# zhm1205/Multimodal_TTA

Hardware: AMD Instinct MI355X
Metric: adapted volumes/sec (higher is better)
Workload: dtype bf16

## Files before the change

### include/mmtta.h

```cpp
#ifndef MMTTA_H
#define MMTTA_H

#include <stdint.h>

#ifdef __cplusplus
extern "C" {
#endif

#define MMTTA_ABI_VERSION 2

typedef enum {
  MMTTA_OK = 0,
  MMTTA_ERR_INVALID = -1,
  MMTTA_ERR_UNSUPPORTED = -2,
  MMTTA_ERR_LAUNCH = -3,
  MMTTA_ERR_WORKSPACE = -4
} mmtta_status;

typedef enum { MMTTA_F32 = 0, MMTTA_BF16 = 1 } mmtta_dtype;

typedef struct {
  void* ptr;
  int32_t n, c, d, h, w;
  int64_t sn, sc, sd, sh, sw;
  int32_t dtype;
  int32_t flags;
} mmtta_tensor;

#define MMTTA_TENSOR_OWNS_PAD 1

#define MMTTA_ACT_NONE 0
#define MMTTA_ACT_RELU 1
#define MMTTA_ACT_LEAKY_RELU 2
typedef struct {
  const float* mean;
  const float* rstd;
  const float* gamma;
  const float* beta;
  int32_t relu;
  int32_t per_item;
  const float* scale;
  const float* shift;
  float negative_slope;
  int32_t _pad2;
} mmtta_norm_on_load;

const char* mmtta_last_error(void);
int mmtta_abi_version(void);

#define MMTTA_OPT_PROFILE_MAIN_KERNEL_ONLY 1
#define MMTTA_OPT_SPLITK_BELOW 2
#define MMTTA_OPT_SPLITK_TARGET 3
#define MMTTA_OPT_WGRAD_WORKGROUPS 4
#define MMTTA_OPT_WGRAD_THIN_SLABS 5
#define MMTTA_OPT_IGEMM_PIPELINE 6
#define MMTTA_OPT_EPILOGUE_VEC16 9
#define MMTTA_OPT_IGEMM_LEAN 10
#define MMTTA_OPT_WGRAD_VECTOR_STAGING 11
#define MMTTA_OPT_CLASS_FUSED_MIN_WORKGROUPS 12
#define MMTTA_OPT_THIN_MFMA 13
#define MMTTA_OPT_IGEMM_FRAGMENT_REUSE 14
#define MMTTA_OPT_LAME_TILED 15
#define MMTTA_OPT_RAW_STAGING 16
#define MMTTA_OPT_HEAD_LOSS_PAIR 17
#define MMTTA_OPT_THIN_LEAN 18
#define MMTTA_OPT_WGRAD_EPILOGUE_UPDATE 19
#define MMTTA_OPT_CLS8_PIPELINE 20
#define MMTTA_OPT_CLS8_LEAN_EPILOGUE 21
int mmtta_set_option(int key, int value);

int mmtta_copy_strided(const mmtta_tensor* src, const mmtta_tensor* dst, void* stream);

typedef enum {
  MMTTA_CONV_FWD = 0,
  MMTTA_CONV_DGRAD = 1,
  MMTTA_CONVT_FWD = 2,
  MMTTA_CONVT_DGRAD = 3
} mmtta_conv_op;

typedef struct {
  int32_t op;
  int32_t ksize;
  int32_t stride;
  int32_t cin;
  int32_t cout;
  int32_t dtype;
} mmtta_conv_desc;

int64_t mmtta_conv_packed_bytes(const mmtta_conv_desc* desc);

int mmtta_conv_pack_weights(const mmtta_conv_desc* desc, const float* w_master, void* packed, void* stream);

typedef struct {
  mmtta_conv_desc desc;
  const float* w_master;
  void* packed;
} mmtta_pack_item;
int64_t mmtta_conv_pack_table_bytes(int count);
int mmtta_conv_pack_table_build(const mmtta_pack_item* items, int count, void* table_host, int64_t* total);
int mmtta_conv_pack_batched(const void* table_dev, int count, int64_t total, void* stream);

typedef struct {
  int32_t tiles;
  int32_t launches;
  int32_t ksplit;
  int32_t stats_rows;
  int32_t config;
  int32_t _pad;
  int64_t workspace_bytes;
} mmtta_conv_plan_t;

int mmtta_conv_plan(const mmtta_conv_desc* desc, const mmtta_tensor* x, const mmtta_tensor* y,
                    mmtta_conv_plan_t* plan);

typedef struct {
  const mmtta_tensor* add;
  mmtta_norm_on_load add_norm;
} mmtta_conv_epilogue;

int mmtta_conv_run(const mmtta_conv_desc* desc, const mmtta_tensor* x, const mmtta_norm_on_load* x_norm,
                   const void* packed, const float* bias, const mmtta_conv_epilogue* epi,
                   const mmtta_tensor* y, int accumulate, float* stats, void* workspace,
                   int64_t workspace_bytes, void* stream);

int mmtta_conv_route(const mmtta_conv_desc* desc, const mmtta_tensor* x, const mmtta_norm_on_load* x_norm,
                     const mmtta_conv_epilogue* epi, const mmtta_tensor* y, int accumulate, const float* stats);

int mmtta_conv_stages_raw(const mmtta_conv_desc* desc, const mmtta_tensor* x, const mmtta_norm_on_load* x_norm,
                          const mmtta_conv_epilogue* epi, const mmtta_tensor* y, int accumulate, const float* stats);

int mmtta_conv_cls8_pipelined(const mmtta_conv_desc* desc, const mmtta_tensor* x, const mmtta_norm_on_load* x_norm,
                              const mmtta_conv_epilogue* epi, const mmtta_tensor* y, int accumulate, const float* stats);

int mmtta_conv_cls8_lean_epilogue(const mmtta_conv_desc* desc, const mmtta_tensor* x, const mmtta_norm_on_load* x_norm,
                                  const mmtta_conv_epilogue* epi, const mmtta_tensor* y, int accumulate, const float* stats);

int mmtta_conv_thin_lean(const mmtta_conv_desc* desc, const mmtta_tensor* x, const mmtta_norm_on_load* x_norm,
                         const mmtta_conv_epilogue* epi, const mmtta_tensor* y, int accumulate, const float* stats);

int mmtta_conv_thin_kernel(const mmtta_conv_desc* desc, const mmtta_tensor* x, const mmtta_norm_on_load* x_norm,
                           const mmtta_conv_epilogue* epi, const mmtta_tensor* y, int accumulate, const float* stats);

typedef struct {
  int32_t items_per_set;
  int32_t inner;
  int64_t packed_outer, packed_inner;
  int64_t weight_outer, weight_inner;
  int64_t bias_outer, bias_inner;
} mmtta_param_sets;

int mmtta_conv_run_sets(const mmtta_conv_desc* desc, const mmtta_tensor* x, const mmtta_norm_on_load* x_norm,
                        const void* packed, const float* bias, const mmtta_conv_epilogue* epi,
                        const mmtta_tensor* y, int accumulate, float* stats, void* workspace,
                        int64_t workspace_bytes, const mmtta_param_sets* sets, void* stream);

int mmtta_conv_head_loss_eligible(const mmtta_conv_desc* desc, const mmtta_tensor* x, const mmtta_norm_on_load* x_norm,
                                  const mmtta_conv_epilogue* epi, const mmtta_tensor* y, const mmtta_tensor* dlogits,
                                  int softmax, int per_item);
int64_t mmtta_conv_head_loss_partials(const mmtta_conv_desc* desc, const mmtta_tensor* x, const mmtta_tensor* y);
int mmtta_conv_head_loss_run_sets(const mmtta_conv_desc* desc, const mmtta_tensor* x, const mmtta_norm_on_load* x_norm,
                                  const void* packed, const float* bias, const mmtta_conv_epilogue* epi,
                                  const mmtta_tensor* y, const mmtta_tensor* dlogits, int softmax, int per_item,
                                  double* partial, float* loss, const mmtta_param_sets* sets, void* stream);

int64_t mmtta_conv_wgrad_workspace_bytes(const mmtta_conv_desc* desc, const mmtta_tensor* x,
                                         const mmtta_tensor* dy);
int mmtta_conv_wgrad_kernel(const mmtta_conv_desc* desc, const mmtta_tensor* x, const mmtta_tensor* dy);
int mmtta_conv_wgrad_stages_raw(const mmtta_conv_desc* desc, const mmtta_tensor* x, const mmtta_norm_on_load* x_norm,
                                const mmtta_tensor* dy);
int mmtta_conv_wgrad(const mmtta_conv_desc* desc, const mmtta_tensor* x, const mmtta_norm_on_load* x_norm,
                     const mmtta_tensor* dy, float* dw, float* db, int accumulate, void* workspace,
                     int64_t workspace_bytes, void* stream);

int64_t mmtta_conv_wgrad_workspace_bytes_sets(const mmtta_conv_desc* desc, const mmtta_tensor* x, const mmtta_tensor* dy,
                                              const mmtta_param_sets* sets);
int mmtta_conv_wgrad_sets(const mmtta_conv_desc* desc, const mmtta_tensor* x, const mmtta_norm_on_load* x_norm,
                          const mmtta_tensor* dy, float* dw, float* db, int accumulate, void* workspace,
                          int64_t workspace_bytes, const mmtta_param_sets* sets, void* stream);
int mmtta_conv_wgrad_plan_sets(const mmtta_conv_desc* desc, const mmtta_tensor* x, const mmtta_tensor* dy,
                               const mmtta_param_sets* sets, int32_t plan[4]);

typedef struct {
  int32_t clip, zscore, masked, min_count;
  float lo, hi, mask_gt, eps;
  float mean, std;
  int32_t legacy, _pad;
} mmtta_intensity_rule;
int64_t mmtta_intensity_scratch_bytes(int channels);
int mmtta_intensity_normalize(const mmtta_tensor* x, const mmtta_intensity_rule* rules, const mmtta_tensor* y,
                              void* scratch, void* stream);

typedef enum {
  MMTTA_NORM_INSTANCE = 0,
  MMTTA_NORM_BATCH = 1,
  MMTTA_NORM_GROUP = 2
} mmtta_norm_kind;

int mmtta_norm_stats_finalize(int kind, int groups, const float* part, int rows_per_n, int n, int c,
                              int64_t count, float eps, int training, float* running_mean,
                              float* running_var, float momentum, float* mean, float* rstd,
                              const float* gamma, const float* beta, float* scale, float* shift,
                              double* scratch, void* stream);

typedef struct {
  int32_t items_per_set;
  int32_t _pad;
  int64_t affine_stride;
  int64_t stats_stride;
} mmtta_norm_sets;

int mmtta_norm_stats_finalize_sets(int kind, int groups, const float* part, int rows_per_n, int n, int c,
                                   int64_t count, float eps, int training, float* running_mean,
                                   float* running_var, float momentum, float* mean, float* rstd,
                                   const float* gamma, const float* beta, float* scale, float* shift,
                                   float* gamma_items, float* beta_items, double* scratch,
                                   const mmtta_norm_sets* sets, void* stream);

int mmtta_reduce_rows_per_n(const mmtta_tensor* t);

int mmtta_channel_stats(const mmtta_tensor* x, float* part, void* stream);

// ... 76 lines not shown
int mmtta_entropy_loss_items(const mmtta_tensor* logits, int softmax, const mmtta_tensor* dlogits,
                             double* partial, float* loss, void* stream);

int64_t mmtta_entropy_filtered_partials(const mmtta_tensor* logits);
int mmtta_entropy_filtered_items(const mmtta_tensor* logits, int softmax, float margin, const uint8_t* keep_in,
                                 uint8_t* keep_out, const mmtta_tensor* dlogits, double* partial, float* loss,
                                 int64_t* kept, void* stream);

int mmtta_mirror_views(const mmtta_tensor* x, const mmtta_tensor* y, int views, const int32_t* view_axes, void* stream);
int64_t mmtta_memo_partials(const mmtta_tensor* logits, int views);
int mmtta_memo_loss_items(const mmtta_tensor* logits, int softmax, int views, const int32_t* view_axes,
                          const mmtta_tensor* dlogits, double* partial, float* loss, void* stream);
int mmtta_memo_ensemble(const mmtta_tensor* logits, int softmax, int views, const int32_t* view_axes,
                        const mmtta_tensor* out, void* stream);

int64_t mmtta_consistency_partials(const mmtta_tensor* logits);
int mmtta_consistency_loss_items(const mmtta_tensor* logits, const mmtta_tensor* target, int softmax,
                                 const mmtta_tensor* dlogits, double* partial, float* loss, void* stream);
int64_t mmtta_cotta_update_partials(int64_t n, int sets);
int mmtta_cotta_update_sets(float* w, float* teacher, const float* source, int64_t n, int sets, int64_t w_stride,
                            int64_t teacher_stride, double alpha, float restore_p, uint64_t seed, const int32_t* step,
                            const int32_t* ordinals, int64_t* partial, int64_t* restored, void* stream);

int mmtta_affine_views(const mmtta_tensor* x, const mmtta_tensor* y, int views, int first, int count,
                       const float* matrices_host, const float* matrices, void* stream);
int mmtta_affine_ensemble(const mmtta_tensor* logits, int softmax, int views, const int32_t* view_axes, int first, int count,
                          const float* inv_host, const float* inv, const mmtta_tensor* out, void* stream);

int mmtta_magnitude_select_class(int64_t length);
int64_t mmtta_magnitude_select_chunks(int64_t length);
int64_t mmtta_magnitude_select_scratch_bytes(int count, int sets);
int mmtta_magnitude_select_sets(const float* g, const int64_t* table, const int64_t* table_host, int count, int sets,
                                int64_t set_stride, uint32_t* gamma_out, void* scratch, void* stream);
int64_t mmtta_petal_update_partials(int64_t n, int sets);
int mmtta_petal_update_sets(float* w, float* teacher, const float* source, const float* g, const uint32_t* gamma,
                            const int64_t* table, const int64_t* table_host, int count, int64_t n, int sets,
                            int64_t w_stride, int64_t teacher_stride, int64_t g_stride, double alpha, int64_t* partial,
                            int64_t* restored, void* stream);

int64_t mmtta_intensity_range_partials(const mmtta_tensor* x);
int mmtta_intensity_range(const mmtta_tensor* x, float* partial, float* range, void* stream);
int mmtta_augment_views(const mmtta_tensor* x, const mmtta_tensor* y, int views, const int32_t* view_axes,
                        const float* table_host, const float* table, const float* range, uint64_t seed,
                        const int32_t* ordinals, void* stream);

int64_t mmtta_entropy_weighted_partials(const mmtta_tensor* logits);
int mmtta_entropy_weighted_items(const mmtta_tensor* logits, int softmax, float margin, uint8_t* keep_out,
                                 const mmtta_tensor* dlogits, double* partial, float* loss, int64_t* kept, void* stream);
int64_t mmtta_pseudo_label_partials(const mmtta_tensor* logits);
int mmtta_pseudo_label_loss_items(const mmtta_tensor* logits, int softmax, const mmtta_tensor* dlogits, double* partial,
                                  float* loss, void* stream);
int mmtta_fisher_accumulate_sets(float* fisher, const float* grads, int64_t n, int sets, int64_t set_stride, void* stream);
int mmtta_fisher_scale(float* fisher, int64_t n, float count, void* stream);
int64_t mmtta_fisher_penalty_partials(int64_t n, int sets);
int mmtta_fisher_penalty_sets(const float* w, float* g, const float* fisher, const float* source, int64_t n, int sets,
                              int replicas, int64_t set_stride, float lambda, double* partial, float* penalty, void* stream);

int mmtta_patch_shuffle(const mmtta_tensor* x, const mmtta_tensor* y, const int32_t* grid, const int32_t* table, void* stream);
int64_t mmtta_deyo_partials(const mmtta_tensor* logits);
int mmtta_deyo_loss_items(const mmtta_tensor* logits, const mmtta_tensor* logits_shuffled, const int32_t* grid,
                          const int32_t* table, int softmax, float margin, float margin0, float plpd_threshold,
                          uint8_t* keep_out, const mmtta_tensor* dlogits, double* partial, float* loss, int64_t* kept,
                          int64_t* kept_entropy, void* stream);

int mmtta_lame_refine(const mmtta_tensor* logits0, const mmtta_tensor* x, uint32_t channel_mask, int softmax, int connectivity,
                      float weight, float sigma, int iterations, const mmtta_tensor* work, const mmtta_tensor* out,
                      int64_t* flipped, void* stream);

int64_t mmtta_crf_partials(const mmtta_tensor* logits);
int mmtta_crf_entropy_items(const mmtta_tensor* logits, const mmtta_tensor* x, uint32_t channel_mask, int softmax,
                            int connectivity, int form, float weight, float sigma, const mmtta_tensor* dlogits,
                            double* partial, float* loss, float* entropy, float* pairwise, void* stream);

int64_t mmtta_nuclear_scratch(const mmtta_tensor* logits, int softmax, int bd, int bh, int bw);
int mmtta_nuclear_entropy_items(const mmtta_tensor* logits, int softmax, int bd, int bh, int bw, float entropy_weight,
                                float weight, float eps, const mmtta_tensor* dlogits, double* scratch, float* loss,
                                float* entropy, float* nuclear, void* stream);

typedef struct mmtta_input_norm_branch {
  const mmtta_tensor* dy;
  const float* weight;
  int64_t set_stride;
  int32_t ksize, stride;
} mmtta_input_norm_branch;
int mmtta_input_norm_apply(const mmtta_tensor* x, const mmtta_tensor* y, const float* theta, const float* range,
                           uint32_t keep_mask, int gamma, void* stream);
int64_t mmtta_input_norm_grad_partials(const mmtta_tensor* x);
int mmtta_input_norm_grad(const mmtta_tensor* x, const mmtta_input_norm_branch* branches, int n_branches, float* theta,
                          const float* range, uint32_t keep_mask, int gamma, double* partial, float* grad, float* exp_avg,
                          float* exp_avg_sq, int32_t* step, double lr, double bound_log_scale, double bound_shift,
                          double bound_log_gamma, void* stream);

#define MMTTA_BIAS_ANCHOR_MIN 0
#define MMTTA_BIAS_ANCHOR_ZERO 1
int mmtta_bias_field_apply(const mmtta_tensor* x, const mmtta_tensor* y, const float* theta, const float* range,
                           const float* tables_d, const float* tables_h, const float* tables_w, int order, int anchor,
                           uint32_t keep_mask, void* stream);
int64_t mmtta_bias_field_grad_partials(const mmtta_tensor* x, int order);
int mmtta_bias_field_grad(const mmtta_tensor* x, const mmtta_input_norm_branch* branches, int n_branches, float* theta,
                          const float* range, const float* tables_d, const float* tables_h, const float* tables_w, int order,
                          int anchor, uint32_t keep_mask, double* partial, float* grad, float* exp_avg, float* exp_avg_sq,
                          int32_t* step, double lr, double bound_gain, double bound_field, double l2, void* stream);

int mmtta_modality_views(const mmtta_tensor* x, const mmtta_tensor* y, int views, const uint32_t* keep_masks, void* stream);
int64_t mmtta_modcons_partials(const mmtta_tensor* logits, int views);
int mmtta_modcons_loss_items(const mmtta_tensor* logits, int softmax, int views, float weight, float entropy_weight, int detach,
                             const mmtta_tensor* dlogits, double* partial, float* loss, float* entropy, float* consistency,
                             float* view_kl, int64_t* disagree, void* stream);

typedef struct mmtta_window_grid {
  int32_t extent[3];
  int32_t count[3];
} mmtta_window_grid;
int mmtta_window_views(const mmtta_tensor* x, const mmtta_tensor* y, const mmtta_window_grid* windows,
                       const int32_t* origins_host, const int32_t* origins, float pad_value, void* stream);
int64_t mmtta_window_partials(const mmtta_tensor* logits);
int mmtta_window_entropy_items(const mmtta_tensor* logits, int softmax, const mmtta_window_grid* windows, const float* tables,
                               const mmtta_tensor* dlogits, double* partial, float* loss, void* stream);
int mmtta_window_blend(const mmtta_tensor* logits, const mmtta_tensor* out, const mmtta_window_grid* windows,
                       const int32_t* origins, const float* tables, void* stream);

int mmtta_adam_step(float* p, const float* g, float* m, float* v, int64_t n, int64_t n_decay, float lr,
                    float beta1, float beta2, float eps, float weight_decay, int32_t* step, void* stream);

enum { MMTTA_OPTIM_ADAM = 0, MMTTA_OPTIM_ADAMW = 1, MMTTA_OPTIM_SGD = 2 };
typedef struct mmtta_optim_desc {
  int32_t kind;
  float lr, beta1, beta2, eps, weight_decay;
  float momentum, dampening;
  int32_t nesterov;
} mmtta_optim_desc;
int mmtta_optim_step(const mmtta_optim_desc* desc, float* p, const float* g, float* m, float* v, int64_t n,
                     int64_t n_decay, int32_t* step, void* stream);

int mmtta_optim_step_sets(const mmtta_optim_desc* desc, float* p, const float* g, float* m, float* v, int64_t n,
                          int64_t n_decay, int sets, int64_t set_stride, int32_t* step, void* stream);

typedef struct mmtta_update_target {
  mmtta_optim_desc optim;
  float* w_p; float* w_m; float* w_v;
  float* b_p; float* b_m; float* b_v;
  float* b_grad;
  void* image[2];
  int64_t image_outer[2], image_inner[2];
  const int32_t* step;
  int32_t w_decay, b_decay;
} mmtta_update_target;
int mmtta_fused_update_enabled(void);
int mmtta_conv_wgrad_update_sets(const mmtta_conv_desc* desc, const mmtta_tensor* x, const mmtta_norm_on_load* x_norm,
                                 const mmtta_tensor* dy, const mmtta_update_target* target, void* workspace,
                                 int64_t workspace_bytes, const mmtta_param_sets* sets, void* stream);
int mmtta_conv_wgrad_updates_in_epilogue(const mmtta_conv_desc* desc, const mmtta_tensor* x, const mmtta_norm_on_load* x_norm,
                                         const mmtta_tensor* dy, const mmtta_param_sets* sets);

int mmtta_optim_step_segments(const mmtta_optim_desc* desc, float* p, const float* g, float* m, float* v, const int64_t* segments,
                              int count, int64_t total, int sets, int64_t set_stride, int32_t* step, void* stream);

int64_t mmtta_sam_ascent_partials(int64_t n, int sets);
int mmtta_sam_ascent_sets(float* p, const float* g, float* saved, int64_t saved_stride, double* partial, int64_t n, int sets,
                          int replicas, int64_t set_stride, float rho, void* stream);

int mmtta_mask_dice_counts(const mmtta_tensor* logits, const mmtta_tensor* label, float threshold,
                           int64_t* counts, uint8_t* mask, void* stream);

int64_t mmtta_dice_ce_scratch_bytes(const mmtta_tensor* logits);
int mmtta_dice_ce_sums(const mmtta_tensor* logits, const mmtta_tensor* label, const float* weight,
                       int squared_pred, int softmax, double* out, void* scratch, void* stream);

int mmtta_dice_ce_grad(const mmtta_tensor* logits, const mmtta_tensor* label, const float* weight, int squared_pred,
                       int softmax, int jaccard, int include_background, float lambda_dice, float lambda_ce, float smooth_nr,
                       float smooth_dr, const double* sums, const mmtta_tensor* dlogits, void* stream);

int64_t mmtta_calibration_scratch_bytes(const mmtta_tensor* logits, int bins);
int mmtta_calibration_bins(const mmtta_tensor* logits, const mmtta_tensor* label, int softmax, int bins, int scope,
                           double* out, void* scratch, void* stream);

int64_t mmtta_components_scratch_bytes(int64_t n_masks, int64_t d, int64_t h, int64_t w);
int mmtta_components_filter(const uint8_t* mask_in, uint8_t* mask_out, const mmtta_tensor* label, int n, int r, int d, int h,
                            int w, int connectivity, const int64_t* min_voxels, const int32_t* keep_largest, int64_t* counts,
                            int64_t* stats, int32_t* labels, void* scratch, void* stream);

int64_t mmtta_lesionwise_scratch_bytes(int64_t n_masks, int64_t d, int64_t h, int64_t w);
int mmtta_lesionwise_scores(const uint8_t* mask, const mmtta_tensor* label, int n, int r, int d, int h, int w, int iterations,
                            int dilation_connectivity, const int64_t* min_lesion_voxels, int64_t* stats, int32_t* labels,
                            void* scratch, void* stream);

int64_t mmtta_lesionwise_hd95_scratch_bytes(int64_t n_masks, int64_t d, int64_t h, int64_t w);
int mmtta_lesionwise_hd95(const uint8_t* mask, const mmtta_tensor* label, int n, int r, int d, int h, int w,
                          const double* spacing, double percentile, const int64_t* min_lesion_voxels,
                          const void* lesionwise_scratch, int64_t* hd_stats, float* lesion_hd,
                          void* scratch, void* stream);

int64_t mmtta_mask_fill_nest_scratch_bytes(int64_t n_masks, int64_t d, int64_t h, int64_t w);
int mmtta_mask_fill_nest(uint8_t* mask, const mmtta_tensor* label, int n, int r, int d, int h, int w, int fill_connectivity,
                         const int32_t* fill_holes, const int64_t* max_hole_voxels, const int32_t* chain, int chain_len,
                         int nest_mode, int64_t* counts, int64_t* stats, void* scratch, void* stream);

int64_t mmtta_surface_scratch_bytes(int64_t n_masks, int64_t d, int64_t h, int64_t w);
int mmtta_surface_distances(const uint8_t* pred_mask, const mmtta_tensor* label, const double* spacing,
                            double percentile, int asd_symmetric, float* hd, float* asd, void* scratch, void* stream);

int64_t mmtta_surface_dice_scratch_bytes(int64_t n_masks, int64_t d, int64_t h, int64_t w);
int mmtta_surface_dice(const uint8_t* pred_mask, const mmtta_tensor* label, const double* spacing, const double* tolerances,
                       int n_tolerances, int64_t* counts, void* scratch, void* stream);

int mmtta_lesionwise_nsd_list_slots(void);
int64_t mmtta_lesionwise_nsd_scratch_bytes(int64_t n_masks, int64_t d, int64_t h, int64_t w);
int mmtta_lesionwise_nsd(const uint8_t* mask, int n, int r, int d, int h, int w, const double* spacing,
                         const double* tolerances, int n_tolerances, const int64_t* min_lesion_voxels,
                         const void* lesionwise_scratch, int64_t* nsd_stats, float* lesion_nsd, void* scratch, void* stream);

#ifdef __cplusplus
}
#endif
#endif
```

### multimodal_tta_amd/_lib.py

```python
from __future__ import annotations

import ctypes as C
import os
from typing import Optional, Sequence

import torch

_HERE = os.path.dirname(os.path.abspath(__file__))
LIB_PATH = os.path.join(_HERE, "csrc", "libmmtta.so")

F32, BF16 = 0, 1
CONV_FWD, CONV_DGRAD, CONVT_FWD, CONVT_DGRAD = 0, 1, 2, 3
NORM_INSTANCE, NORM_BATCH, NORM_GROUP = 0, 1, 2


class MmttaError(RuntimeError):
    pass


class Tensor(C.Structure):
    _fields_ = [
        ("ptr", C.c_void_p),
        ("n", C.c_int32), ("c", C.c_int32), ("d", C.c_int32), ("h", C.c_int32), ("w", C.c_int32),
        ("sn", C.c_int64), ("sc", C.c_int64), ("sd", C.c_int64), ("sh", C.c_int64), ("sw", C.c_int64),
# ... 92 lines not shown
    "mmtta_last_error": (C.c_char_p, []),
    "mmtta_abi_version": (C.c_int, []),
    "mmtta_set_option": (C.c_int, [C.c_int, C.c_int]),
    "mmtta_intensity_scratch_bytes": (C.c_int64, [C.c_int]),
    "mmtta_intensity_normalize": (C.c_int, [_P(Tensor), _P(IntensityRule), _P(Tensor), C.c_void_p, C.c_void_p]),
    "mmtta_copy_strided": (C.c_int, [_P(Tensor), _P(Tensor), C.c_void_p]),
    "mmtta_conv_packed_bytes": (C.c_int64, [_P(ConvDesc)]),
    "mmtta_conv_pack_weights": (C.c_int, [_P(ConvDesc), C.c_void_p, C.c_void_p, C.c_void_p]),
    "mmtta_conv_pack_table_bytes": (C.c_int64, [C.c_int]),
    "mmtta_conv_pack_table_build": (C.c_int, [_P(PackItem), C.c_int, C.c_void_p, _P(C.c_int64)]),
    "mmtta_conv_pack_batched": (C.c_int, [C.c_void_p, C.c_int, C.c_int64, C.c_void_p]),
    "mmtta_conv_plan": (C.c_int, [_P(ConvDesc), _P(Tensor), _P(Tensor), _P(ConvPlan)]),
    "mmtta_conv_run": (C.c_int, [_P(ConvDesc), _P(Tensor), _P(NormOnLoad), C.c_void_p, C.c_void_p, _P(ConvEpilogue),
                                 _P(Tensor), C.c_int, C.c_void_p, C.c_void_p, C.c_int64, C.c_void_p]),
    "mmtta_conv_run_sets": (C.c_int, [_P(ConvDesc), _P(Tensor), _P(NormOnLoad), C.c_void_p, C.c_void_p, _P(ConvEpilogue),
                                      _P(Tensor), C.c_int, C.c_void_p, C.c_void_p, C.c_int64, _P(ParamSets), C.c_void_p]),
    "mmtta_conv_route": (C.c_int, [_P(ConvDesc), _P(Tensor), _P(NormOnLoad), _P(ConvEpilogue), _P(Tensor), C.c_int, C.c_void_p]),
    "mmtta_conv_stages_raw": (C.c_int, [_P(ConvDesc), _P(Tensor), _P(NormOnLoad), _P(ConvEpilogue), _P(Tensor), C.c_int, C.c_void_p]),
    "mmtta_conv_cls8_pipelined": (C.c_int, [_P(ConvDesc), _P(Tensor), _P(NormOnLoad), _P(ConvEpilogue), _P(Tensor), C.c_int, C.c_void_p]),
    "mmtta_conv_cls8_lean_epilogue": (C.c_int, [_P(ConvDesc), _P(Tensor), _P(NormOnLoad), _P(ConvEpilogue), _P(Tensor), C.c_int, C.c_void_p]),
    "mmtta_conv_thin_lean": (C.c_int, [_P(ConvDesc), _P(Tensor), _P(NormOnLoad), _P(ConvEpilogue), _P(Tensor), C.c_int, C.c_void_p]),
    "mmtta_conv_thin_kernel": (C.c_int, [_P(ConvDesc), _P(Tensor), _P(NormOnLoad), _P(ConvEpilogue), _P(Tensor), C.c_int, C.c_void_p]),
    "mmtta_conv_head_loss_eligible": (C.c_int, [_P(ConvDesc), _P(Tensor), _P(NormOnLoad), _P(ConvEpilogue), _P(Tensor), _P(Tensor),
                                                C.c_int, C.c_int]),
    "mmtta_conv_head_loss_partials": (C.c_int64, [_P(ConvDesc), _P(Tensor), _P(Tensor)]),
    "mmtta_conv_head_loss_run_sets": (C.c_int, [_P(ConvDesc), _P(Tensor), _P(NormOnLoad), C.c_void_p, C.c_void_p, _P(ConvEpilogue),
                                                _P(Tensor), _P(Tensor), C.c_int, C.c_int, C.c_void_p, C.c_void_p, _P(ParamSets),
                                                C.c_void_p]),
    "mmtta_conv_wgrad_workspace_bytes": (C.c_int64, [_P(ConvDesc), _P(Tensor), _P(Tensor)]),
    "mmtta_conv_wgrad_workspace_bytes_sets": (C.c_int64, [_P(ConvDesc), _P(Tensor), _P(Tensor), _P(ParamSets)]),
    "mmtta_conv_wgrad_plan_sets": (C.c_int, [_P(ConvDesc), _P(Tensor), _P(Tensor), _P(ParamSets), _P(C.c_int32)]),
    "mmtta_conv_wgrad_sets": (C.c_int, [_P(ConvDesc), _P(Tensor), _P(NormOnLoad), _P(Tensor), C.c_void_p, C.c_void_p,
                                        C.c_int, C.c_void_p, C.c_int64, _P(ParamSets), C.c_void_p]),
    "mmtta_conv_wgrad_kernel": (C.c_int, [_P(ConvDesc), _P(Tensor), _P(Tensor)]),
    "mmtta_conv_wgrad_stages_raw": (C.c_int, [_P(ConvDesc), _P(Tensor), _P(NormOnLoad), _P(Tensor)]),
    "mmtta_conv_wgrad": (C.c_int, [_P(ConvDesc), _P(Tensor), _P(NormOnLoad), _P(Tensor), C.c_void_p, C.c_void_p,
                                   C.c_int, C.c_void_p, C.c_int64, C.c_void_p]),
    "mmtta_norm_stats_finalize": (C.c_int, [C.c_int, C.c_int, C.c_void_p, C.c_int, C.c_int, C.c_int, C.c_int64,
                                            C.c_float, C.c_int, C.c_void_p, C.c_void_p, C.c_float, C.c_void_p,
                                            C.c_void_p, C.c_void_p, C.c_void_p, C.c_void_p, C.c_void_p, C.c_void_p,
                                            C.c_void_p]),
    "mmtta_norm_stats_finalize_sets": (C.c_int, [C.c_int, C.c_int, C.c_void_p, C.c_int, C.c_int, C.c_int, C.c_int64,
                                                 C.c_float, C.c_int, C.c_void_p, C.c_void_p, C.c_float, C.c_void_p,
                                                 C.c_void_p, C.c_void_p, C.c_void_p, C.c_void_p, C.c_void_p, C.c_void_p,
                                                 C.c_void_p, C.c_void_p, _P(NormSets), C.c_void_p]),
    "mmtta_reduce_rows_per_n": (C.c_int, [_P(Tensor)]),
    "mmtta_channel_stats": (C.c_int, [_P(Tensor), C.c_void_p, C.c_void_p]),
    "mmtta_combine": (C.c_int, [_P(Tensor), _P(NormOnLoad), _P(Tensor), _P(NormOnLoad), _P(Tensor), C.c_void_p]),
    "mmtta_norm_bwd_reduce": (C.c_int, [_P(Tensor), _P(Tensor), _P(NormOnLoad), C.c_void_p, C.c_void_p]),
    "mmtta_norm_bwd_finalize": (C.c_int, [C.c_int, C.c_int, C.c_void_p, C.c_int, C.c_int, C.c_int, C.c_int64,
                                          C.c_void_p, C.c_int, C.c_void_p, C.c_void_p, C.c_void_p, C.c_void_p,
                                          C.c_int, C.c_void_p, C.c_void_p]),
    "mmtta_norm_bwd_finalize_sets": (C.c_int, [C.c_int, C.c_int, C.c_void_p, C.c_int, C.c_int, C.c_int, C.c_int64,
                                               C.c_void_p, C.c_int, C.c_void_p, C.c_void_p, C.c_void_p, C.c_void_p,
                                               C.c_int, C.c_void_p, _P(NormSets), C.c_void_p]),
    "mmtta_norm_bwd_apply": (C.c_int, [_P(Tensor), _P(Tensor), _P(NormOnLoad), C.c_void_p, C.c_void_p, _P(Tensor),
                                       C.c_void_p]),
    "mmtta_norm_bwd_small_ok": (C.c_int, [_P(Tensor), _P(Tensor), _P(NormOnLoad), _P(Tensor)]),
    "mmtta_norm_bwd_small": (C.c_int, [_P(Tensor), _P(Tensor), _P(NormOnLoad), C.c_int64, _P(Tensor), C.c_void_p]),
    "mmtta_upsample2x_fwd": (C.c_int, [_P(Tensor), _P(Tensor), C.c_void_p]),
    "mmtta_upsample2x_bwd": (C.c_int, [_P(Tensor), _P(Tensor), C.c_int, C.c_void_p]),
    "mmtta_lincomb": (C.c_int, [C.c_int, _P(_P(Tensor)), _P(C.c_float), _P(Tensor), C.c_int, C.c_void_p]),
    "mmtta_pointwise_route": (C.c_int, [C.c_int, _P(_P(Tensor)), C.c_int, _P(NormOnLoad), _P(NormOnLoad), C.c_void_p, C.c_void_p,
                                        _P(PointwiseRoute)]),
    "mmtta_entropy_partials": (C.c_int64, [_P(Tensor)]),
    "mmtta_entropy_loss": (C.c_int, [_P(Tensor), C.c_int, _P(Tensor), C.c_void_p, C.c_void_p, C.c_void_p]),
    "mmtta_entropy_partials_items": (C.c_int64, [_P(Tensor)]),
    "mmtta_entropy_loss_items": (C.c_int, [_P(Tensor), C.c_int, _P(Tensor), C.c_void_p, C.c_void_p, C.c_void_p]),
    "mmtta_entropy_filtered_partials": (C.c_int64, [_P(Tensor)]),
    "mmtta_entropy_filtered_items": (C.c_int, [_P(Tensor), C.c_int, C.c_float, C.c_void_p, C.c_void_p, _P(Tensor), C.c_void_p,
                                               C.c_void_p, C.c_void_p, C.c_void_p]),
    "mmtta_mirror_views": (C.c_int, [_P(Tensor), _P(Tensor), C.c_int, _P(C.c_int32), C.c_void_p]),
    "mmtta_memo_partials": (C.c_int64, [_P(Tensor), C.c_int]),
    "mmtta_memo_loss_items": (C.c_int, [_P(Tensor), C.c_int, C.c_int, _P(C.c_int32), _P(Tensor), C.c_void_p, C.c_void_p,
                                        C.c_void_p]),
    "mmtta_memo_ensemble": (C.c_int, [_P(Tensor), C.c_int, C.c_int, _P(C.c_int32), _P(Tensor), C.c_void_p]),
    "mmtta_affine_views": (C.c_int, [_P(Tensor), _P(Tensor), C.c_int, C.c_int, C.c_int, C.c_void_p, C.c_void_p, C.c_void_p]),
    "mmtta_affine_ensemble": (C.c_int, [_P(Tensor), C.c_int, C.c_int, _P(C.c_int32), C.c_int, C.c_int, C.c_void_p, C.c_void_p,
                                        _P(Tensor), C.c_void_p]),
    "mmtta_consistency_partials": (C.c_int64, [_P(Tensor)]),
    "mmtta_consistency_loss_items": (C.c_int, [_P(Tensor), _P(Tensor), C.c_int, _P(Tensor), C.c_void_p, C.c_void_p, C.c_void_p]),
    "mmtta_cotta_update_partials": (C.c_int64, [C.c_int64, C.c_int]),
    "mmtta_cotta_update_sets": (C.c_int, [C.c_void_p, C.c_void_p, C.c_void_p, C.c_int64, C.c_int, C.c_int64, C.c_int64,
                                          C.c_double, C.c_float, C.c_uint64, C.c_void_p, C.c_void_p, C.c_void_p, C.c_void_p,
                                          C.c_void_p]),
    "mmtta_magnitude_select_class": (C.c_int, [C.c_int64]),
    "mmtta_magnitude_select_chunks": (C.c_int64, [C.c_int64]),
    "mmtta_magnitude_select_scratch_bytes": (C.c_int64, [C.c_int, C.c_int]),
    "mmtta_magnitude_select_sets": (C.c_int, [C.c_void_p, C.c_void_p, C.c_void_p, C.c_int, C.c_int, C.c_int64, C.c_void_p,
                                              C.c_void_p, C.c_void_p]),
    "mmtta_petal_update_partials": (C.c_int64, [C.c_int64, C.c_int]),
    "mmtta_petal_update_sets": (C.c_int, [C.c_void_p, C.c_void_p, C.c_void_p, C.c_void_p, C.c_void_p, C.c_void_p, C.c_void_p,
                                          C.c_int, C.c_int64, C.c_int, C.c_int64, C.c_int64, C.c_int64, C.c_double, C.c_void_p,
                                          C.c_void_p, C.c_void_p]),
    "mmtta_intensity_range_partials": (C.c_int64, [_P(Tensor)]),
    "mmtta_intensity_range": (C.c_int, [_P(Tensor), C.c_void_p, C.c_void_p, C.c_void_p]),
    "mmtta_augment_views": (C.c_int, [_P(Tensor), _P(Tensor), C.c_int, _P(C.c_int32), C.c_void_p, C.c_void_p, C.c_void_p,
                                      C.c_uint64, C.c_void_p, C.c_void_p]),
    "mmtta_entropy_weighted_partials": (C.c_int64, [_P(Tensor)]),
    "mmtta_entropy_weighted_items": (C.c_int, [_P(Tensor), C.c_int, C.c_float, C.c_void_p, _P(Tensor), C.c_void_p, C.c_void_p,
                                               C.c_void_p, C.c_void_p]),
    "mmtta_pseudo_label_partials": (C.c_int64, [_P(Tensor)]),
    "mmtta_pseudo_label_loss_items": (C.c_int, [_P(Tensor), C.c_int, _P(Tensor), C.c_void_p, C.c_void_p, C.c_void_p]),
    "mmtta_fisher_accumulate_sets": (C.c_int, [C.c_void_p, C.c_void_p, C.c_int64, C.c_int, C.c_int64, C.c_void_p]),
    "mmtta_fisher_scale": (C.c_int, [C.c_void_p, C.c_int64, C.c_float, C.c_void_p]),
    "mmtta_fisher_penalty_partials": (C.c_int64, [C.c_int64, C.c_int]),
    "mmtta_fisher_penalty_sets": (C.c_int, [C.c_void_p, C.c_void_p, C.c_void_p, C.c_void_p, C.c_int64, C.c_int, C.c_int,
                                            C.c_int64, C.c_float, C.c_void_p, C.c_void_p, C.c_void_p]),
    "mmtta_patch_shuffle": (C.c_int, [_P(Tensor), _P(Tensor), _P(C.c_int32), C.c_void_p, C.c_void_p]),
    "mmtta_deyo_partials": (C.c_int64, [_P(Tensor)]),
    "mmtta_deyo_loss_items": (C.c_int, [_P(Tensor), _P(Tensor), _P(C.c_int32), C.c_void_p, C.c_int, C.c_float, C.c_float,
                                        C.c_float, C.c_void_p, _P(Tensor), C.c_void_p, C.c_void_p, C.c_void_p, C.c_void_p,
                                        C.c_void_p]),
    "mmtta_lame_refine": (C.c_int, [_P(Tensor), _P(Tensor), C.c_uint32, C.c_int, C.c_int, C.c_float, C.c_float, C.c_int,
                                    _P(Tensor), _P(Tensor), C.c_void_p, C.c_void_p]),
    "mmtta_crf_partials": (C.c_int64, [_P(Tensor)]),
    "mmtta_crf_entropy_items": (C.c_int, [_P(Tensor), _P(Tensor), C.c_uint32, C.c_int, C.c_int, C.c_int, C.c_float, C.c_float,
                                          _P(Tensor), C.c_void_p, C.c_void_p, C.c_void_p, C.c_void_p, C.c_void_p]),
    "mmtta_nuclear_scratch": (C.c_int64, [_P(Tensor), C.c_int, C.c_int, C.c_int, C.c_int]),
    "mmtta_nuclear_entropy_items": (C.c_int, [_P(Tensor), C.c_int, C.c_int, C.c_int, C.c_int, C.c_float, C.c_float, C.c_float,
                                              _P(Tensor), C.c_void_p, C.c_void_p, C.c_void_p, C.c_void_p, C.c_void_p]),
    "mmtta_input_norm_apply": (C.c_int, [_P(Tensor), _P(Tensor), C.c_void_p, C.c_void_p, C.c_uint32, C.c_int, C.c_void_p]),
    "mmtta_input_norm_grad_partials": (C.c_int64, [_P(Tensor)]),
    "mmtta_input_norm_grad": (C.c_int, [_P(Tensor), _P(InputNormBranch), C.c_int, C.c_void_p, C.c_void_p, C.c_uint32, C.c_int,
                                        C.c_void_p, C.c_void_p, C.c_void_p, C.c_void_p, C.c_void_p, C.c_double, C.c_double,
                                        C.c_double, C.c_double, C.c_void_p]),
    "mmtta_bias_field_apply": (C.c_int, [_P(Tensor), _P(Tensor), C.c_void_p, C.c_void_p, C.c_void_p, C.c_void_p, C.c_void_p, C.c_int,
                                         C.c_int, C.c_uint32, C.c_void_p]),
    "mmtta_bias_field_grad_partials": (C.c_int64, [_P(Tensor), C.c_int]),
    "mmtta_bias_field_grad": (C.c_int, [_P(Tensor), _P(InputNormBranch), C.c_int, C.c_void_p, C.c_void_p, C.c_void_p, C.c_void_p,
                                        C.c_void_p, C.c_int, C.c_int, C.c_uint32, C.c_void_p, C.c_void_p, C.c_void_p, C.c_void_p,
                                        C.c_void_p, C.c_double, C.c_double, C.c_double, C.c_double, C.c_void_p]),
    "mmtta_modality_views": (C.c_int, [_P(Tensor), _P(Tensor), C.c_int, _P(C.c_uint32), C.c_void_p]),
    "mmtta_modcons_partials": (C.c_int64, [_P(Tensor), C.c_int]),
    "mmtta_modcons_loss_items": (C.c_int, [_P(Tensor), C.c_int, C.c_int, C.c_float, C.c_float, C.c_int, _P(Tensor), C.c_void_p,
                                           C.c_void_p, C.c_void_p, C.c_void_p, C.c_void_p, C.c_void_p, C.c_void_p]),
    "mmtta_window_views": (C.c_int, [_P(Tensor), _P(Tensor), _P(WindowGrid), _P(C.c_int32), C.c_void_p, C.c_float, C.c_void_p]),
    "mmtta_window_partials": (C.c_int64, [_P(Tensor)]),
    "mmtta_window_entropy_items": (C.c_int, [_P(Tensor), C.c_int, _P(WindowGrid), C.c_void_p, _P(Tensor), C.c_void_p, C.c_void_p,
                                             C.c_void_p]),
    "mmtta_window_blend": (C.c_int, [_P(Tensor), _P(Tensor), _P(WindowGrid), C.c_void_p, C.c_void_p, C.c_void_p]),
    "mmtta_adam_step": (C.c_int, [C.c_void_p, C.c_void_p, C.c_void_p, C.c_void_p, C.c_int64, C.c_int64, C.c_float,
                                  C.c_float, C.c_float, C.c_float, C.c_float, C.c_void_p, C.c_void_p]),
    "mmtta_optim_step": (C.c_int, [_P(OptimDesc), C.c_void_p, C.c_void_p, C.c_void_p, C.c_void_p, C.c_int64, C.c_int64,
                                   C.c_void_p, C.c_void_p]),
    "mmtta_optim_step_sets": (C.c_int, [_P(OptimDesc), C.c_void_p, C.c_void_p, C.c_void_p, C.c_void_p, C.c_int64, C.c_int64,
                                        C.c_int, C.c_int64, C.c_void_p, C.c_void_p]),
    "mmtta_optim_step_segments": (C.c_int, [_P(OptimDesc), C.c_void_p, C.c_void_p, C.c_void_p, C.c_void_p, C.c_void_p, C.c_int,
                                            C.c_int64, C.c_int, C.c_int64, C.c_void_p, C.c_void_p]),
    "mmtta_fused_update_enabled": (C.c_int, []),
    "mmtta_conv_wgrad_update_sets": (C.c_int, [_P(ConvDesc), _P(Tensor), _P(NormOnLoad), _P(Tensor), _P(UpdateTarget),
                                               C.c_void_p, C.c_int64, _P(ParamSets), C.c_void_p]),
    "mmtta_conv_wgrad_updates_in_epilogue": (C.c_int, [_P(ConvDesc), _P(Tensor), _P(NormOnLoad), _P(Tensor), _P(ParamSets)]),
    "mmtta_sam_ascent_partials": (C.c_int64, [C.c_int64, C.c_int]),
    "mmtta_sam_ascent_sets": (C.c_int, [C.c_void_p, C.c_void_p, C.c_void_p, C.c_int64, C.c_void_p, C.c_int64, C.c_int, C.c_int,
                                        C.c_int64, C.c_float, C.c_void_p]),
    "mmtta_mask_dice_counts": (C.c_int, [_P(Tensor), _P(Tensor), C.c_float, C.c_void_p, C.c_void_p, C.c_void_p]),
    "mmtta_dice_ce_scratch_bytes": (C.c_int64, [_P(Tensor)]),
    "mmtta_dice_ce_sums": (C.c_int, [_P(Tensor), _P(Tensor), C.c_void_p, C.c_int, C.c_int, C.c_void_p, C.c_void_p, C.c_void_p]),
    "mmtta_dice_ce_grad": (C.c_int, [_P(Tensor), _P(Tensor), C.c_void_p, C.c_int, C.c_int, C.c_int, C.c_int, C.c_float, C.c_float,
                                     C.c_float, C.c_float, C.c_void_p, _P(Tensor), C.c_void_p]),
    "mmtta_calibration_scratch_bytes": (C.c_int64, [_P(Tensor), C.c_int]),
    "mmtta_calibration_bins": (C.c_int, [_P(Tensor), _P(Tensor), C.c_int, C.c_int, C.c_int, C.c_void_p, C.c_void_p, C.c_void_p]),
    "mmtta_components_scratch_bytes": (C.c_int64, [C.c_int64, C.c_int64, C.c_int64, C.c_int64]),
    "mmtta_components_filter": (C.c_int, [C.c_void_p, C.c_void_p, _P(Tensor), C.c_int, C.c_int, C.c_int, C.c_int, C.c_int, C.c_int,
                                          _P(C.c_int64), _P(C.c_int32), C.c_void_p, C.c_void_p, C.c_void_p, C.c_void_p, C.c_void_p]),
    "mmtta_lesionwise_scratch_bytes": (C.c_int64, [C.c_int64, C.c_int64, C.c_int64, C.c_int64]),
    "mmtta_lesionwise_scores": (C.c_int, [C.c_void_p, _P(Tensor), C.c_int, C.c_int, C.c_int, C.c_int, C.c_int, C.c_int, C.c_int,
                                          _P(C.c_int64), C.c_void_p, C.c_void_p, C.c_void_p, C.c_void_p]),
    "mmtta_lesionwise_hd95_scratch_bytes": (C.c_int64, [C.c_int64, C.c_int64, C.c_int64, C.c_int64]),
    "mmtta_lesionwise_hd95": (C.c_int, [C.c_void_p, _P(Tensor), C.c_int, C.c_int, C.c_int, C.c_int, C.c_int, _P(C.c_double), C.c_double,
                                        _P(C.c_int64), C.c_void_p, C.c_void_p, C.c_void_p, C.c_void_p, C.c_void_p]),
    "mmtta_mask_fill_nest_scratch_bytes": (C.c_int64, [C.c_int64, C.c_int64, C.c_int64, C.c_int64]),
    "mmtta_mask_fill_nest": (C.c_int, [C.c_void_p, _P(Tensor), C.c_int, C.c_int, C.c_int, C.c_int, C.c_int, C.c_int, _P(C.c_int32),
                                       _P(C.c_int64), _P(C.c_int32), C.c_int, C.c_int, C.c_void_p, C.c_void_p, C.c_void_p, C.c_void_p]),
    "mmtta_surface_scratch_bytes": (C.c_int64, [C.c_int64, C.c_int64, C.c_int64, C.c_int64]),
    "mmtta_surface_distances": (C.c_int, [C.c_void_p, _P(Tensor), _P(C.c_double), C.c_double, C.c_int, C.c_void_p,
                                          C.c_void_p, C.c_void_p, C.c_void_p]),
    "mmtta_surface_dice_scratch_bytes": (C.c_int64, [C.c_int64, C.c_int64, C.c_int64, C.c_int64]),
    "mmtta_surface_dice": (C.c_int, [C.c_void_p, _P(Tensor), _P(C.c_double), _P(C.c_double), C.c_int, C.c_void_p, C.c_void_p,
                                     C.c_void_p]),
    "mmtta_lesionwise_nsd_list_slots": (C.c_int, []),
    "mmtta_lesionwise_nsd_scratch_bytes": (C.c_int64, [C.c_int64, C.c_int64, C.c_int64, C.c_int64]),
    "mmtta_lesionwise_nsd": (C.c_int, [C.c_void_p, C.c_int, C.c_int, C.c_int, C.c_int, C.c_int, _P(C.c_double), _P(C.c_double),
                                       C.c_int, _P(C.c_int64), C.c_void_p, C.c_void_p, C.c_void_p, C.c_void_p, C.c_void_p]),
}

_lib = None


def load() -> C.CDLL:
    global _lib
    if _lib is not None:
        return _lib
    if not os.path.exists(LIB_PATH):
        raise MmttaError(
            f"{LIB_PATH} is missing: build it with `python -m multimodal_tta_amd.build` (hipcc, gfx950). "
            "There is no CPU or PyTorch fallback for the adaptation path."
        )
    lib = C.CDLL(LIB_PATH)
    for name, (res, args) in _SIGNATURES.items():
        fn = getattr(lib, name)
        fn.restype = res
        fn.argtypes = args
    if lib.mmtta_abi_version() != 2:
        raise MmttaError("libmmtta.so ABI version mismatch")
    if os.environ.get("MMTTA_NO_PIPE", "0") == "1":
        lib.mmtta_set_option(6, 0)
    if os.environ.get("MMTTA_NO_EPIVEC", "0") == "1":
        lib.mmtta_set_option(9, 0)
    if "MMTTA_WGVEC" in os.environ:
        lib.mmtta_set_option(11, int(os.environ["MMTTA_WGVEC"]))
    if "MMTTA_THINMFMA" in os.environ:
        lib.mmtta_set_option(13, int(os.environ["MMTTA_THINMFMA"]))
    if "MMTTA_CLSFUSE" in os.environ:
        lib.mmtta_set_option(12, int(os.environ["MMTTA_CLSFUSE"]))
    if "MMTTA_LEAN" in os.environ:
        lib.mmtta_set_option(10, int(os.environ["MMTTA_LEAN"]))
    if "MMTTA_RAWSTAGE" in os.environ:
        lib.mmtta_set_option(16, int(os.environ["MMTTA_RAWSTAGE"]))
    if "MMTTA_HEADLOSS" in os.environ:
        lib.mmtta_set_option(17, int(os.environ["MMTTA_HEADLOSS"]))
    if "MMTTA_THINLEAN" in os.environ:
        lib.mmtta_set_option(18, int(os.environ["MMTTA_THINLEAN"]))
    if "MMTTA_EPIUPDATE" in os.environ:
        lib.mmtta_set_option(19, int(os.environ["MMTTA_EPIUPDATE"]))
    if "MMTTA_CLS8PIPE" in os.environ:
        lib.mmtta_set_option(20, int(os.environ["MMTTA_CLS8PIPE"]))
    if "MMTTA_CLS8LEAN" in os.environ:
        lib.mmtta_set_option(21, int(os.environ["MMTTA_CLS8LEAN"]))
    _lib = lib
    return lib


def exported_names() -> Sequence[str]:
    return list(_SIGNATURES)


def check(status: int, what: str = "") -> None:
    if status != 0:
        msg = load().mmtta_last_error().decode("utf-8", "replace")
        raise MmttaError(f"{what or 'libmmtta'} failed with status {status}: {msg}")


def stream_ptr() -> int:
    return int(torch.cuda.current_stream().cuda_stream)


def ptr(t: Optional[torch.Tensor]) -> Optional[int]:
    return None if t is None else int(t.data_ptr())


TENSOR_OWNS_PAD = 1


def desc_cl(t: torch.Tensor) -> Tensor:
    if t.dim() != 5 or t.dtype not in (torch.float32, torch.bfloat16) or not t.is_cuda:
        raise MmttaError(f"expected a CUDA float32 / bfloat16 [N,D,H,W,C] view, got {tuple(t.shape)} {t.dtype} {t.device}")
    n, d, h, w, c = t.shape
    sn, sd, sh, sw, sc = t.stride()
    if sc != 1 and c != 1:
        raise MmttaError("activation views must have unit stride along C")
    flags = TENSOR_OWNS_PAD if getattr(t, "_mmtta_owns_pad", False) else 0
    return Tensor(t.data_ptr(), n, c, d, h, w, sn, 1, sd, sh, sw, BF16 if t.dtype == torch.bfloat16 else F32, flags)


def desc_ncdhw(t: torch.Tensor) -> Tensor:
    if t.dim() != 5 or t.dtype != torch.float32 or not t.is_cuda:
        raise MmttaError(f"expected a CUDA float32 [N,C,D,H,W] tensor, got {tuple(t.shape)} {t.dtype} {t.device}")
    n, c, d, h, w = t.shape
    sn, sc, sd, sh, sw = t.stride()
    return Tensor(t.data_ptr(), n, c, d, h, w, sn, sc, sd, sh, sw, F32, 0)


ACT_NONE, ACT_RELU, ACT_LEAKY_RELU = 0, 1, 2


def norm_on_load(mean=None, rstd=None, gamma=None, beta=None, relu=False, scale=None, shift=None,
                 per_item=False, act=None, negative_slope=0.0) -> NormOnLoadAct:
    code = (ACT_RELU if relu else ACT_NONE) if act is None else int(act)
    return NormOnLoadAct(ptr(mean), ptr(rstd), ptr(gamma), ptr(beta), code, 1 if per_item else 0, ptr(scale),
                      ptr(shift), float(negative_slope) if code == ACT_LEAKY_RELU else 0.0, 0)
```

### multimodal_tta_amd/csrc/api.hip

```cpp
#include "common.h"
#include <string.h>

namespace mmtta {
static thread_local char g_err[512] = "";
void set_error(const char* fmt, ...) {
  va_list ap;
  va_start(ap, fmt);
  vsnprintf(g_err, sizeof(g_err), fmt, ap);
  va_end(ap);
}
int g_profile_main_only = 0;
int g_igemm_pipeline = 1;
int g_epilogue_vec = 1;
int g_igemm_lean = 1;
int g_igemm_reuse = 1;
int g_cls_fused_min = 128;
int g_thin_mfma = 2;
int g_wgrad_vec = 1;
int g_lame_tiled = 1;
int g_raw_staging = 3;
int g_head_loss_pair = 3;
int g_thin_lean = 3;
int g_wgrad_epilogue_update = 1;
int g_cls8_pipeline = 1;
int g_cls8_lean_epilogue = 1;
int g_tune[4] = {96, 128, 128, 256};
}

extern "C" int mmtta_set_option(int key, int value) {
  if (key == MMTTA_OPT_PROFILE_MAIN_KERNEL_ONLY) {
    const int prev = mmtta::g_profile_main_only;
    mmtta::g_profile_main_only = value;
    return prev;
  }
  if (key == MMTTA_OPT_WGRAD_VECTOR_STAGING) {
    const int prev = mmtta::g_wgrad_vec;
    mmtta::g_wgrad_vec = value ? 1 : 0;
    return prev;
  }
  if (key == MMTTA_OPT_THIN_MFMA) {
    const int prev = mmtta::g_thin_mfma;
    mmtta::g_thin_mfma = value < 0 ? 0 : (value > 3 ? 3 : value);
    return prev;
  }
  if (key == MMTTA_OPT_CLASS_FUSED_MIN_WORKGROUPS) {
    const int prev = mmtta::g_cls_fused_min;
    mmtta::g_cls_fused_min = value < 0 ? 0 : value;
    return prev;
  }
  if (key == MMTTA_OPT_IGEMM_LEAN) {
    const int prev = mmtta::g_igemm_lean;
    mmtta::g_igemm_lean = value ? 1 : 0;
    return prev;
  }
  if (key == MMTTA_OPT_IGEMM_FRAGMENT_REUSE) {
    const int prev = mmtta::g_igemm_reuse;
    mmtta::g_igemm_reuse = value ? 1 : 0;
    return prev;
  }
  if (key == MMTTA_OPT_EPILOGUE_VEC16) {
    const int prev = mmtta::g_epilogue_vec;
    mmtta::g_epilogue_vec = value ? 1 : 0;
    return prev;
  }
  if (key == MMTTA_OPT_LAME_TILED) {
    const int prev = mmtta::g_lame_tiled;
    mmtta::g_lame_tiled = value ? 1 : 0;
    return prev;
  }
  if (key == MMTTA_OPT_RAW_STAGING) {
    const int prev = mmtta::g_raw_staging;
    mmtta::g_raw_staging = value & 3;
    return prev;
  }
  if (key == MMTTA_OPT_HEAD_LOSS_PAIR) {
    const int prev = mmtta::g_head_loss_pair;
    mmtta::g_head_loss_pair = value & 3;
    return prev;
  }
  if (key == MMTTA_OPT_THIN_LEAN) {
    const int prev = mmtta::g_thin_lean;
    mmtta::g_thin_lean = value & 3;
    return prev;
  }
  if (key == MMTTA_OPT_WGRAD_EPILOGUE_UPDATE) {
    const int prev = mmtta::g_wgrad_epilogue_update;
    mmtta::g_wgrad_epilogue_update = value ? 1 : 0;
    return prev;
  }
  if (key == MMTTA_OPT_CLS8_PIPELINE) {
    const int prev = mmtta::g_cls8_pipeline;
    mmtta::g_cls8_pipeline = value ? 1 : 0;
    return prev;
  }
  if (key == MMTTA_OPT_CLS8_LEAN_EPILOGUE) {
    const int prev = mmtta::g_cls8_lean_epilogue;
    mmtta::g_cls8_lean_epilogue = value & 1;
    return prev;
  }
  if (key == MMTTA_OPT_IGEMM_PIPELINE) {
    const int prev = mmtta::g_igemm_pipeline;
    mmtta::g_igemm_pipeline = value ? 1 : 0;
    return prev;
  }
  if (key >= MMTTA_OPT_SPLITK_BELOW && key <= MMTTA_OPT_WGRAD_THIN_SLABS) {
    if (value < 1) return MMTTA_ERR_INVALID;
    const int prev = mmtta::g_tune[key - MMTTA_OPT_SPLITK_BELOW];
    mmtta::g_tune[key - MMTTA_OPT_SPLITK_BELOW] = value;
    return prev;
  }
  return MMTTA_ERR_INVALID;
}

extern "C" const char* mmtta_last_error(void) { return mmtta::g_err; }
extern "C" int mmtta_abi_version(void) { return MMTTA_ABI_VERSION; }
```

### multimodal_tta_amd/csrc/common.h

```cpp
#pragma once
#include <hip/hip_runtime.h>
#include <type_traits>
#include <stdint.h>
#include <stdio.h>
#include <stdarg.h>
#include "../../include/mmtta.h"

namespace mmtta {

constexpr int WAVE = 64;

void set_error(const char* fmt, ...);

#define MMTTA_CHECK(cond, code, ...)      \
  do {                                    \
    if (!(cond)) {                        \
      ::mmtta::set_error(__VA_ARGS__);    \
      return (code);                      \
    }                                     \
  } while (0)

inline int launch_status(const char* what) {
  hipError_t e = hipGetLastError();
  if (e != hipSuccess) {
    set_error("%s: %s", what, hipGetErrorString(e));
    return MMTTA_ERR_LAUNCH;
  }
  return MMTTA_OK;
}

extern int g_profile_main_only;
extern int g_igemm_pipeline;
extern int g_wgrad_vec;
extern int g_igemm_lean;
extern int g_igemm_reuse;
extern int g_cls_fused_min;
extern int g_lame_tiled;
extern int g_thin_mfma;
extern int g_epilogue_vec;
extern int g_raw_staging;
extern int g_head_loss_pair;
extern int g_thin_lean;
extern int g_wgrad_epilogue_update;
extern int g_cls8_pipeline;
extern int g_cls8_lean_epilogue;
extern int g_tune[4];

inline bool nl_leaky(const mmtta_norm_on_load* t) { return t != nullptr && t->relu == MMTTA_ACT_LEAKY_RELU; }
inline int nl_act_check(const mmtta_norm_on_load* t, const char* what) {
  MMTTA_CHECK(t == nullptr || (t->relu >= MMTTA_ACT_NONE && t->relu <= MMTTA_ACT_LEAKY_RELU), MMTTA_ERR_INVALID,
              "%s: activation code %d (MMTTA_ACT_NONE, _RELU or _LEAKY_RELU)", what, t ? t->relu : 0);
  MMTTA_CHECK(t == nullptr || t->relu != MMTTA_ACT_LEAKY_RELU || __builtin_isfinite(t->negative_slope), MMTTA_ERR_INVALID,
              "%s: LeakyReLU negative_slope must be finite", what);
  return MMTTA_OK;
}

struct PackImageGeo {
  int A, B, T, Kp, Np, kn_is_ba, plain_bf16;
};
int pack_image_geometry(const mmtta_conv_desc* d, PackImageGeo& g);

#define MMTTA_ACT_BODIES                                                                                                    \
  int conv_run_body(const mmtta_conv_desc* d, const mmtta_tensor* x, const mmtta_norm_on_load* x_norm, const void* packed,  \
                    const float* bias, const mmtta_conv_epilogue* epi, const mmtta_tensor* y, int accumulate, float* stats, \
                    void* workspace, int64_t workspace_bytes, const mmtta_param_sets* sets, void* stream);                \
  int conv_wgrad_body(const mmtta_conv_desc* d, const mmtta_tensor* x, const mmtta_norm_on_load* x_norm,                    \
                      const mmtta_tensor* dy, float* dw, float* db, int accumulate, void* workspace,                        \
                      int64_t workspace_bytes, const mmtta_param_sets* sets, void* stream,                                  \
                      const mmtta_update_target* upd);                                                                      \
  int combine_body(const mmtta_tensor* a, const mmtta_norm_on_load* ta, const mmtta_tensor* b,                              \
                   const mmtta_norm_on_load* tb, const mmtta_tensor* out, void* stream);                                    \
  int norm_bwd_reduce_body(const mmtta_tensor* dout, const mmtta_tensor* y, const mmtta_norm_on_load* t, float* part,      \
                           void* stream);                                                                                   \
  int norm_bwd_apply_body(const mmtta_tensor* dout, const mmtta_tensor* y, const mmtta_norm_on_load* t, const float* m1,   \
                          const float* m2, const mmtta_tensor* dy, void* stream);                                           \
  int norm_bwd_small_body(const mmtta_tensor* dout, const mmtta_tensor* y, const mmtta_norm_on_load* t, int64_t count,     \
                          const mmtta_tensor* dy, void* stream);
namespace leaky { MMTTA_ACT_BODIES }

#ifdef MMTTA_ACT_LEAKY_TU
#define MMTTA_ACT_NS_OPEN namespace leaky {
#define MMTTA_ACT_NS_CLOSE }
#else
#define MMTTA_ACT_NS_OPEN
#define MMTTA_ACT_NS_CLOSE
#endif

MMTTA_ACT_NS_OPEN
MMTTA_ACT_BODIES

inline bool is_cl(const mmtta_tensor* t) { return t->sc == 1 || t->c == 1; }

inline bool is_f32(const mmtta_tensor* t) { return t->dtype == MMTTA_F32; }
inline bool is_bf16(const mmtta_tensor* t) { return t->dtype == MMTTA_BF16; }

inline bool quad_aligned(const mmtta_tensor* t, int base_bytes, int elems = 4) {
  return ((uintptr_t)t->ptr) % base_bytes == 0 && t->sw % elems == 0 && t->sh % elems == 0 && t->sd % elems == 0 &&
         t->sn % elems == 0;
}
inline int quad_bytes(const mmtta_tensor* t) { return is_bf16(t) ? 8 : 16; }
inline bool item_fits_31(const mmtta_tensor* t, int64_t pad) {
  const int64_t last = (int64_t)(t->d - 1) * t->sd + (int64_t)(t->h - 1) * t->sh + (int64_t)(t->w - 1) * t->sw + pad;
  return last < ((int64_t)1 << 31);
}
inline bool strides_fit_24(const mmtta_tensor* t) { return t->sw < (1 << 24) && t->sh < (1 << 24) && t->sd < (1 << 24); }
inline bool voxel_dense(const mmtta_tensor* t) { return t->sc == 1 && t->sh == (int64_t)t->w * t->sw && t->sd == (int64_t)t->h * t->sh; }
inline bool dense_rows16(const mmtta_tensor* t) {
  const int q = is_bf16(t) ? 8 : 4;
  return voxel_dense(t) && ((uintptr_t)t->ptr) % 16 == 0 && t->sw % q == 0 && t->sn % q == 0 &&
         (int64_t)t->d * t->h * t->w * t->sw < ((int64_t)1 << 31);
}
inline bool same_shape(const mmtta_tensor* a, const mmtta_tensor* b) {
  return a->n == b->n && a->c == b->c && a->d == b->d && a->h == b->h && a->w == b->w;
}

__device__ __forceinline__ float bf16_bits_to_f32(unsigned int h) { return __uint_as_float(h << 16); }
__device__ __forceinline__ unsigned int f32x2_to_bf16x2(float lo, float hi) {
  typedef __bf16 bf2 __attribute__((ext_vector_type(2)));
  bf2 v;
  v[0] = (__bf16)lo;
  v[1] = (__bf16)hi;
  return __builtin_bit_cast(unsigned int, v);
}
__device__ __forceinline__ unsigned short f32_to_bf16_bits(float v) { return __builtin_bit_cast(unsigned short, (__bf16)v); }
__device__ __forceinline__ uint4 bf16x8_pack(const unsigned short* h) {
  uint4 q;
  q.x = h[0] | ((unsigned)h[1] << 16); q.y = h[2] | ((unsigned)h[3] << 16);
  q.z = h[4] | ((unsigned)h[5] << 16); q.w = h[6] | ((unsigned)h[7] << 16);
  return q;
}
__device__ __forceinline__ float4 ld4_any(const float* base, long long eoff, int bf) {
  if (bf) {
    const uint2 u = *reinterpret_cast<const uint2*>(reinterpret_cast<const unsigned short*>(base) + eoff);
    return make_float4(bf16_bits_to_f32(u.x & 0xffffu), bf16_bits_to_f32(u.x >> 16), bf16_bits_to_f32(u.y & 0xffffu),
                       bf16_bits_to_f32(u.y >> 16));
  }
  return *reinterpret_cast<const float4*>(base + eoff);
}
__device__ __forceinline__ void st4_any(float* base, long long eoff, float4 v, int bf) {
  if (bf) {
    uint2 u;
    u.x = f32x2_to_bf16x2(v.x, v.y);
    u.y = f32x2_to_bf16x2(v.z, v.w);
    *reinterpret_cast<uint2*>(reinterpret_cast<unsigned short*>(base) + eoff) = u;
  } else {
    *reinterpret_cast<float4*>(base + eoff) = v;
  }
}
__device__ __forceinline__ float ld1_any(const float* base, long long eoff, int bf) {
  if (bf) return bf16_bits_to_f32(reinterpret_cast<const unsigned short*>(base)[eoff]);
  return base[eoff];
}
__device__ __forceinline__ void st1_any(float* base, long long eoff, float v, int bf) {
  if (bf) reinterpret_cast<unsigned short*>(base)[eoff] = (unsigned short)(f32x2_to_bf16x2(v, 0.f) & 0xffffu);
  else base[eoff] = v;
}
__device__ __forceinline__ void ld8_any(const float* base, long long eoff, int bf, float4& lo, float4& hi) {
  if (bf) {
    const uint4 u = *reinterpret_cast<const uint4*>(reinterpret_cast<const unsigned short*>(base) + eoff);
    lo = make_float4(bf16_bits_to_f32(u.x & 0xffffu), bf16_bits_to_f32(u.x >> 16), bf16_bits_to_f32(u.y & 0xffffu),
                     bf16_bits_to_f32(u.y >> 16));
    hi = make_float4(bf16_bits_to_f32(u.z & 0xffffu), bf16_bits_to_f32(u.z >> 16), bf16_bits_to_f32(u.w & 0xffffu),
                     bf16_bits_to_f32(u.w >> 16));
  } else {
    lo = *reinterpret_cast<const float4*>(base + eoff);
    hi = *reinterpret_cast<const float4*>(base + eoff + 4);
  }
}

template <bool BF> struct Oct8 { float4 lo, hi; };
template <> struct Oct8<true> { uint4 q; };
template <bool BF>
__device__ __forceinline__ Oct8<BF> oct8_ld(const float* base, unsigned eoff_lo, unsigned eoff_hi) {
  Oct8<BF> o;
  if constexpr (BF) {
    o.q = *reinterpret_cast<const uint4*>(reinterpret_cast<const unsigned short*>(base) + eoff_lo);
  } else {
    o.lo = *reinterpret_cast<const float4*>(base + eoff_lo);
    o.hi = *reinterpret_cast<const float4*>(base + eoff_hi);
  }
  return o;
}
__device__ __forceinline__ void oct8_f8(const Oct8<false>& o, float (&v)[8]) {
  v[0] = o.lo.x; v[1] = o.lo.y; v[2] = o.lo.z; v[3] = o.lo.w; v[4] = o.hi.x; v[5] = o.hi.y; v[6] = o.hi.z; v[7] = o.hi.w;
}
__device__ __forceinline__ void oct8_f8(const Oct8<true>& o, float (&v)[8]) {
  v[0] = bf16_bits_to_f32(o.q.x & 0xffffu); v[1] = __uint_as_float(o.q.x & 0xffff0000u);
  v[2] = bf16_bits_to_f32(o.q.y & 0xffffu); v[3] = __uint_as_float(o.q.y & 0xffff0000u);
  v[4] = bf16_bits_to_f32(o.q.z & 0xffffu); v[5] = __uint_as_float(o.q.z & 0xffff0000u);
  v[6] = bf16_bits_to_f32(o.q.w & 0xffffu); v[7] = __uint_as_float(o.q.w & 0xffff0000u);
}


template <bool BF>
__device__ __forceinline__ void oct8_st(float* base, unsigned eoff, const float (&v)[8]) {
  if constexpr (BF) {
    uint4 q;
// ... 349 lines not shown
```

### multimodal_tta_amd/csrc/conv_wgrad.hip

```cpp
#include "common.h"

namespace mmtta {
MMTTA_ACT_NS_OPEN

typedef float f32x16 __attribute__((ext_vector_type(16)));
static inline int roundup(int v, int m) { return (v + m - 1) / m * m; }

struct WArgs {
  const float* g; long long gsn, gsd, gsh, gsw; int Cg, Dgg, Hgg, Wgg; NL tg;
  const float* dn; long long dsn, dsd, dsh, dsw; int Cd, Dd, Hd, Wd; NL td;
  int N;
  int si, ntaps;
  float* slab;
  float* dbpart;
  int tz, ty, tx, tiles, tiles_per_split;
  int S, tiles_set;
  int CGp, CDp;
  int gvec4, dvec4;
  int g_bf, d_bf;
  int convt;
};

template <int TZ, int TY, int TX, int NTW, bool GBF = false, bool DBF = false>
__global__ __launch_bounds__(256) void wgrad_f32_kernel(WArgs a) {
// ... 430 lines not shown
    const float t = bias_rows_sum(dbpart + (long long)q * db_nsl * CDp, db_nsl, Cd, CDp, cd0, tile);
    const float step_size = s_step_size, bc2_sqrt = s_bc2_sqrt;
    const int cd = cd0 + (int)threadIdx.x;
    if (threadIdx.x < 32 && cd < Cd) {
      const long long o = pset_bias_elems(ps, q) + cd;
      float pi = u.bp[o], mi = 0.f, vi = 0.f;
      if (!first) {
        if (keep_m) mi = u.bm[o];
        if (KIND != 2) vi = u.bv[o];
      }
      optim_update<KIND>(pi, t, mi, vi, wd_on && u.b_decay, u.a, step_size, bc2_sqrt, first);
      u.bp[o] = pi;
      if (keep_m) u.bm[o] = mi;
      if (KIND != 2) u.bv[o] = vi;
    }
    return;
  }
  const int cg0 = blockIdx.x * UPD_CG;
  const long long st = (long long)27 * CGp * CDp;
  if (ptr16(slab) && CDp % 4 == 0) {
    upd_reduce4<4>(slab, nsl, st, 0, cg0, cd0, Cg, Cd, CGp, CDp, tile);
    upd_reduce4<3>(slab, nsl, st, 4, cg0, cd0, Cg, Cd, CGp, CDp, tile);
  } else {
    constexpr int NI = 9;
#pragma unroll 1
    for (int j0 = 0; j0 < 27; j0 += NI) {
      const float* pit[NI];
      bool live[NI];
#pragma unroll
      for (int it = 0; it < NI; ++it) {
        const int e = threadIdx.x + 256 * (j0 + it);
        const int cgl = e / 864, i = e % 864, cdl = i & 31, tap = i >> 5;
        const int cg = cg0 + cgl, cd = cd0 + cdl;
        live[it] = cg < Cg && cd < Cd;
        pit[it] = slab + ((long long)tap * CGp + min(cg, Cg - 1)) * CDp + min(cd, CDp - 1);
      }
      float acc[NI];
      slab_sums<NI>(pit, nsl, st, acc);
#pragma unroll
      for (int it = 0; it < NI; ++it) {
        const int e = threadIdx.x + 256 * (j0 + it);
        const int cgl = e / 864, i = e % 864, cdl = i & 31, tap = i >> 5;
        tile[cdl * UPD_RS + cgl * 27 + tap] = live[it] ? acc[it] : 0.f;
      }
    }
  }
  __syncthreads();
  {
    const float step_size = s_step_size, bc2_sqrt = s_bc2_sqrt;
    const bool decay = wd_on && u.w_decay;
    const long long wo = pset_weight_elems(ps, q);
    const int ncg = min(UPD_CG, Cg - cg0);
    const long long ob = wo + ((long long)cd0 * Cg + cg0) * 27, rowst = (long long)Cg * 27;
    bool vec = ncg == UPD_CG && rowst % 4 == 0 && ptr16(u.wp + ob);
    if (keep_m) vec = vec && ptr16(u.wm + ob);
    if (KIND != 2) vec = vec && ptr16(u.wv + ob);
    if (vec) {
      upd_optim4<KIND, 4>(u, ob, rowst, 0, cd0, Cd, first, keep_m, decay, step_size, bc2_sqrt, tile);
      upd_optim4<KIND, 3>(u, ob, rowst, 4, cd0, Cd, first, keep_m, decay, step_size, bc2_sqrt, tile);
    } else {
      for (int e = threadIdx.x; e < UPD_CD * UPD_CG * 27; e += 256) {
        const int cdl = e / (UPD_CG * 27), r = e % (UPD_CG * 27);
        const int cd = cd0 + cdl;
        if (cd < Cd && r < ncg * 27) {
          const long long o = ob + cdl * rowst + r;
          float pi = u.wp[o], mi = 0.f, vi = 0.f;
          if (!first) {
            if (keep_m) mi = u.wm[o];
            if (KIND != 2) vi = u.wv[o];
          }
          optim_update<KIND>(pi, tile[cdl * UPD_RS + r], mi, vi, decay, u.a, step_size, bc2_sqrt, first);
          u.wp[o] = pi;
          if (keep_m) u.wm[o] = mi;
          if (KIND != 2) u.wv[o] = vi;
          tile[cdl * UPD_RS + r] = pi;
        }
      }
    }
  }
  __syncthreads();
#pragma unroll
  for (int m = 0; m < 2; ++m) upd_repack(u.img[m], ps, q, cg0, cd0, tile);
}

__global__ __launch_bounds__(256) void wgrad_reduce1_kernel(const float* __restrict__ slab, float* __restrict__ dw,
                                                            int nsl, int Cg, int Cd, int CGp, int CDp, int accumulate, PSets ps) {
  __shared__ float tile[32][33];
  slab += (long long)blockIdx.z * nsl * CGp * CDp;
  dw += pset_weight_elems(ps, blockIdx.z);
  const int cg0 = blockIdx.x * 32, cd0 = blockIdx.y * 32;
  for (int i = threadIdx.x; i < 32 * 32; i += 256) {
    const int cdl = i & 31, cgl = i >> 5;
    float s = 0.f;
    if (cg0 + cgl < Cg && cd0 + cdl < Cd)
      for (int sl = 0; sl < nsl; ++sl) s += slab[((long long)sl * CGp + cg0 + cgl) * CDp + cd0 + cdl];
    tile[cdl][cgl] = s;
  }
  __syncthreads();
  for (int i = threadIdx.x; i < 32 * 32; i += 256) {
    const int cgl = i & 31, cdl = i >> 5;
    if (cg0 + cgl < Cg && cd0 + cdl < Cd) {
      const long long idx = (long long)(cd0 + cdl) * Cg + cg0 + cgl;
      const float v = tile[cdl][cgl];
      dw[idx] = accumulate ? (dw[idx] + v) : v;
    }
  }
}

__global__ __launch_bounds__(256) void slab_prereduce_kernel(const float* __restrict__ slab, float* __restrict__ out,
                                                             int nsl, long long elems) {
  const long long e = (long long)blockIdx.x * 256 + threadIdx.x;
  if (e >= elems) return;
  slab += (long long)blockIdx.z * nsl * elems;
  out += (long long)blockIdx.z * gridDim.y * elems;
  const int s0 = blockIdx.y * 32, s1 = min(nsl, s0 + 32);
  float acc[8] = {0.f, 0.f, 0.f, 0.f, 0.f, 0.f, 0.f, 0.f};
  for (int sl = s0; sl < s1; sl += 8) {
    float v[8];
#pragma unroll
    for (int u = 0; u < 8; ++u) v[u] = slab[(long long)min(sl + u, s1 - 1) * elems + e];
#pragma unroll
    for (int u = 0; u < 8; ++u) acc[u] += sl + u < s1 ? v[u] : 0.f;
  }
  out[(long long)blockIdx.y * elems + e] = ((acc[0] + acc[1]) + (acc[2] + acc[3])) + ((acc[4] + acc[5]) + (acc[6] + acc[7]));
}

__global__ __launch_bounds__(64) void db_reduce_kernel(const float* __restrict__ part, float* __restrict__ db, int nsl,
                                                       int C, int ld, int accumulate, PSets ps, int is_weight) {
  const int c = blockIdx.x;
  part += (long long)blockIdx.y * nsl * ld;
  db += is_weight ? pset_weight_elems(ps, blockIdx.y) : pset_bias_elems(ps, blockIdx.y);
  float s = 0.f;
  for (int sl = threadIdx.x; sl < nsl; sl += 64) s += part[(long long)sl * ld + c];
  s = wave_sum(s);
  if (threadIdx.x == 0) db[c] = accumulate ? db[c] + s : s;
}

typedef __bf16 wbf16x8 __attribute__((ext_vector_type(8)));
typedef __bf16 wbf16x2 __attribute__((ext_vector_type(2)));
__device__ __forceinline__ unsigned int wpack2(float lo, float hi) {
  wbf16x2 v; v[0] = (__bf16)lo; v[1] = (__bf16)hi;
  return __builtin_bit_cast(unsigned int, v);
}


template <int TZ, int TY, int SI>
struct WTGeo {
  static constexpr int BZ = (TZ - 1) * SI + 3, BY = (TY - 1) * SI + 3, BX = 7 * SI + 3;
  static constexpr int XH = (BX + 1) / 2;
  static constexpr int NG = BZ * BY * BX, ND = TZ * TY * 8;
  static constexpr int G_BYTES = NG * 64, D_BYTES = ND * 64;
  static constexpr int LDS_BYTES = G_BYTES + D_BYTES + 256;
  __host__ __device__ static constexpr int lds_bytes(int nb) { return G_BYTES + nb * (D_BYTES + 256); }
  static constexpr int NK = ND / 16;
  static constexpr int IPR = BX * 4;
  static constexpr int RPP = 256 / IPR;
  static constexpr int NROW = BZ * BY;
  static constexpr int GP = NROW / RPP;
  static constexpr int DP = ND * 4 / 256;
  static_assert(NROW % RPP == 0 && (ND * 4) % 256 == 0 && RPP <= BY, "whole passes; at most one y wrap inside a pass");
  __host__ __device__ static constexpr int xmap(int x) { return SI == 1 ? x : (x & 1) * XH + (x >> 1); }
  __host__ __device__ static constexpr int tap_off(int tap) {
    return (((tap / 9) * BY + (tap / 3) % 3) * BX + xmap(tap % 3)) * 64;
  }
  __host__ __device__ static constexpr int row_off(int ks) {
    return ((((2 * ks) / TY) * SI * BY + ((2 * ks) % TY) * SI) * BX) * 64;
  }
};

typedef short wshort4 __attribute__((ext_vector_type(4)));
typedef short wshort8 __attribute__((ext_vector_type(8)));
typedef __attribute__((address_space(3))) wshort4* wlds4_t;

#define MMTTA_TR_FRAG(ptr, off)                                                                          \
  __builtin_bit_cast(wbf16x8, __builtin_shufflevector(__builtin_amdgcn_ds_read_tr16_b64_v4i16((wlds4_t)((ptr) + (off))),       \
                                                      __builtin_amdgcn_ds_read_tr16_b64_v4i16((wlds4_t)((ptr) + (off) + 256)), \
                                                      0, 1, 2, 3, 4, 5, 6, 7))

#define MMTTA_TR_NO_UPDATE    \
  constexpr bool UPD = false; \
  constexpr int KIND = 0;     \
  constexpr UpdArgs u{};      \
  constexpr PSets ps{};
template <int TZ, int TY, int SI, bool GBF, bool DBF, bool TD, int NB = 1>
__global__ __launch_bounds__(256, (NB == 1 && SI == 1) ? 2 : 1) void wgrad_tr_kernel(WArgs a) {
  constexpr bool RG = false, RD = false;
  MMTTA_TR_NO_UPDATE
#include "conv_wgrad_tr_body.h"
}

template <int TZ, int TY, int SI, bool TD, int NB, bool RG, bool RD>
__global__ __launch_bounds__(256, (NB == 1 && SI == 1) ? 2 : 1) void wgrad_tr_raw_kernel(WArgs a) {
  constexpr bool GBF = true, DBF = true;
  MMTTA_TR_NO_UPDATE
#include "conv_wgrad_tr_body.h"
}

template <int TZ, int TY, int SI, bool TD, int NB, bool RG, bool RD, int KIND>
__global__ __launch_bounds__(256, (NB == 1 && SI == 1) ? 2 : 1) void wgrad_tr_upd_kernel(WArgs a, UpdArgs u, PSets ps) {
  constexpr bool GBF = true, DBF = true, UPD = true;
#include "conv_wgrad_tr_body.h"
}

template <int TZ, int TY, int SI, bool GBF, bool DBF, bool TD, int NB = 1, bool RG = false, bool RD = false>
static int launch_wgrad_tr_t(const WArgs& a, int S, hipStream_t s) {
  using G = WTGeo<TZ, TY, SI>;
  void (*kern)(WArgs);
  if constexpr (RG || RD) kern = wgrad_tr_raw_kernel<TZ, TY, SI, TD, NB, RG, RD>;
  else kern = wgrad_tr_kernel<TZ, TY, SI, GBF, DBF, TD, NB>;
  static bool attr_set = false;
  if (!attr_set) {
    (void)hipFuncSetAttribute((const void*)kern, hipFuncAttributeMaxDynamicSharedMemorySize, 160 * 1024);
    attr_set = true;
  }
  MMTTA_CHECK((a.CDp / 32) % NB == 0, MMTTA_ERR_INVALID, "wgrad: %d dense column blocks in groups of %d", a.CDp / 32, NB);
  dim3 grid(S, a.CGp / 32, a.CDp / 32 / NB);
  hipLaunchKernelGGL(kern, grid, dim3(256), G::lds_bytes(NB), s, a);
  return launch_status("conv wgrad bf16 (transposed reads)");
}

template <bool GBF, bool DBF>
__global__ __launch_bounds__(256, 2) void wgrad_tr1_kernel(WArgs a) {
  constexpr int TZ = 4, TY = 8, NV = TZ * TY * 8, NP = NV * 4 / 256;
  extern __shared__ float lds[];
  unsigned char* gl = reinterpret_cast<unsigned char*>(lds);
  unsigned char* dl = gl + NV * 64;
  float* coefl = reinterpret_cast<float*>(dl + NV * 64);
  const int tid = threadIdx.x, lane = tid & 63;
  const int wave = __builtin_amdgcn_readfirstlane(tid >> 6);
  const int h = lane >> 5, r = lane & 31;
  const int cg0 = blockIdx.y * 32, cd0 = blockIdx.z * 32;
  const int lq = (lane & 15) >> 2, lp = lane & 3, lc = (lane >> 4) & 1;
  const unsigned char* gread = gl + (h * 8 + lq) * 64 + lc * 32 + lp * 8;
  const unsigned char* dread = dl + (h * 8 + lq) * 64 + lc * 32 + lp * 8;
  f32x16 acc;
#pragma unroll
  for (int i = 0; i < 16; ++i) acc[i] = 0.f;
  float dbs[8];
#pragma unroll
  for (int c = 0; c < 8; ++c) dbs[c] = 0.f;
  const bool want_db = a.dbpart != nullptr && blockIdx.y == 0;
  const bool td = a.convt != 0;

  const int vox0 = tid >> 2, c8 = tid & 3;
  unsigned char* gst = gl + vox0 * 64 + c8 * 16;
  unsigned char* dst = dl + vox0 * 64 + c8 * 16;
  const int yl = vox0 >> 3, xl = vox0 & 7;
  const int gcb = cg0 + 8 * c8, dcb = cd0 + 8 * c8;
  const unsigned gc_lo = GBF ? min(gcb, (a.Cg - 1) & ~7) : min(gcb, (a.Cg - 1) & ~3), gc_hi = min(gcb + 4, (a.Cg - 1) & ~3);
  const unsigned dc_lo = DBF ? min(dcb, (a.Cd - 1) & ~7) : min(dcb, (a.Cd - 1) & ~3), dc_hi = min(dcb + 4, (a.Cd - 1) & ~3);
  const bool gtail = (a.Cg & 7) != 0, dtail = (a.Cd & 7) != 0;
  auto pair_mask = [](int c, int C) { return (c < C ? 0xffffu : 0u) | (c + 1 < C ? 0xffff0000u : 0u); };
  const unsigned gsd = (unsigned)a.gsd, gsh = (unsigned)a.gsh, gsw = (unsigned)a.gsw;
  const unsigned dsd = (unsigned)a.dsd, dsh = (unsigned)a.dsh, dsw = (unsigned)a.dsw;

  const int sx = (int)xcd_contiguous_id(blockIdx.x, gridDim.x);
  const int qset = sx / a.S, sls = sx - qset * a.S;
  const int t0 = qset * a.tiles_set + sls * a.tiles_per_split;
  const int t1 = min((qset + 1) * a.tiles_set, t0 + a.tiles_per_split);
  const int tpn = a.tz * a.ty * a.tx;
  Oct8<GBF> gv[NP];
  Oct8<DBF> dq[NP];
  unsigned okbits = 0u;
  int pn = -1, cn = -1;
  auto issue = [&](int tile) {
    pn = tile / tpn;
    int t = tile % tpn;
    const int txi = t % a.tx; t /= a.tx;
    const int tyi = t % a.ty;
    const int tzi = t / a.ty;
    const int oz0 = tzi * TZ, oy = tyi * TY + yl, ox = txi * 8 + xl;
    const float* gbase = reinterpret_cast<const float*>(reinterpret_cast<const char*>(a.g) + (long long)pn * a.gsn * (GBF ? 2 : 4));
    const float* dbase = reinterpret_cast<const float*>(reinterpret_cast<const char*>(a.dn) + (long long)pn * a.dsn * (DBF ? 2 : 4));
    const bool yxok = oy < a.Hd && ox < a.Wd;
    const unsigned gyx = __umul24((unsigned)min(oy, a.Hd - 1), gsh) + __umul24((unsigned)min(ox, a.Wd - 1), gsw);
    const unsigned dyx = __umul24((unsigned)min(oy, a.Hd - 1), dsh) + __umul24((unsigned)min(ox, a.Wd - 1), dsw);
    okbits = 0u;
#pragma unroll
    for (int p = 0; p < NP; ++p) {
      const int oz = oz0 + p;
      okbits |= ((yxok && oz < a.Dd) ? 1u : 0u) << p;
      const unsigned go = __umul24((unsigned)min(oz, a.Dd - 1), gsd) + gyx, dof = __umul24((unsigned)min(oz, a.Dd - 1), dsd) + dyx;
      gv[p] = oct8_ld<GBF>(gbase, go + gc_lo, go + gc_hi);
      dq[p] = oct8_ld<DBF>(dbase, dof + dc_lo, dof + dc_hi);
    }
  };
  if (t0 < t1) issue(t0);
  for (int tile = t0; tile < t1; ++tile) {
    const int n = pn;
    if (n != cn) {
      float s8[8], h8[8];
      if (td) nl_coeff_vec<8>(a.td, n, a.Cd, dcb, s8, h8);
      else nl_coeff_vec<8>(a.tg, n, a.Cg, gcb, s8, h8);
#pragma unroll
      for (int j = 0; j < 8; ++j) { coefl[8 * c8 + j] = s8[j]; coefl[32 + 8 * c8 + j] = h8[j]; }
      cn = n;
      __syncthreads();
    }
    float sc[8], sh[8];
    {
      const float4* cq = reinterpret_cast<const float4*>(coefl + 8 * c8);
      const float4 s0 = cq[0], s1 = cq[1], h0 = cq[8], h1 = cq[9];
      sc[0] = s0.x; sc[1] = s0.y; sc[2] = s0.z; sc[3] = s0.w; sc[4] = s1.x; sc[5] = s1.y; sc[6] = s1.z; sc[7] = s1.w;
      sh[0] = h0.x; sh[1] = h0.y; sh[2] = h0.z; sh[3] = h0.w; sh[4] = h1.x; sh[5] = h1.y; sh[6] = h1.z; sh[7] = h1.w;
    }
    const float relu_lo = act_lo(td ? a.td.relu : a.tg.relu);
#pragma unroll
    for (int p = 0; p < NP; ++p) {
      const unsigned okm = ((okbits >> p) & 1u) ? 0xffffffffu : 0u;
      float v[8], u[8];
      oct8_f8(gv[p], v);
      oct8_f8(dq[p], u);
      if (td) {
#pragma unroll
        for (int j = 0; j < 8; ++j) u[j] = act_max(fmaf(u[j], sc[j], sh[j]), relu_lo);
      } else {
#pragma unroll
        for (int j = 0; j < 8; ++j) v[j] = act_max(fmaf(v[j], sc[j], sh[j]), relu_lo);
      }
      if (want_db) {
#pragma unroll
        for (int j = 0; j < 8; ++j) dbs[j] += __uint_as_float(__float_as_uint(u[j]) & ((dcb + j < a.Cd) ? okm : 0u));
      }
      uint4 pk, pd;
      pk.x = wpack2(v[0], v[1]) & okm; pk.y = wpack2(v[2], v[3]) & okm; pk.z = wpack2(v[4], v[5]) & okm; pk.w = wpack2(v[6], v[7]) & okm;
      pd.x = wpack2(u[0], u[1]) & okm; pd.y = wpack2(u[2], u[3]) & okm; pd.z = wpack2(u[4], u[5]) & okm; pd.w = wpack2(u[6], u[7]) & okm;
      if (gtail) { pk.x &= pair_mask(gcb, a.Cg); pk.y &= pair_mask(gcb + 2, a.Cg); pk.z &= pair_mask(gcb + 4, a.Cg); pk.w &= pair_mask(gcb + 6, a.Cg); }
      if (dtail) { pd.x &= pair_mask(dcb, a.Cd); pd.y &= pair_mask(dcb + 2, a.Cd); pd.z &= pair_mask(dcb + 4, a.Cd); pd.w &= pair_mask(dcb + 6, a.Cd); }
      *reinterpret_cast<uint4*>(gst + p * 4096) = pk;
      *reinterpret_cast<uint4*>(dst + p * 4096) = pd;
    }
    __syncthreads();
    if (tile + 1 < t1) issue(tile + 1);
    wbf16x8 fa[4], fb[4];
#pragma unroll
    for (int i = 0; i < 4; ++i) {
      fa[i] = MMTTA_TR_FRAG(gread, (wave + 4 * i) * 1024);
      fb[i] = MMTTA_TR_FRAG(dread, (wave + 4 * i) * 1024);
    }
#pragma unroll
    for (int i = 0; i < 4; ++i) acc = __builtin_amdgcn_mfma_f32_32x32x16_bf16(fa[i], fb[i], acc, 0, 0, 0);
    __syncthreads();
  }
  const int sl = sx * 4 + wave;
  {
    float* sb = a.slab + ((long long)sl * a.CGp + cg0) * a.CDp + cd0 + r;
#pragma unroll
    for (int i = 0; i < 16; ++i) {
      const int row = (i & 3) + 8 * (i >> 2) + 4 * h;
      sb[(long long)row * a.CDp] = acc[i];
    }
  }
  if (want_db) {
    float* red8 = lds;
#pragma unroll
    for (int c = 0; c < 8; ++c) red8[tid * 8 + c] = dbs[c];
    __syncthreads();
    if (tid < 32) {
      float sacc = 0.f;
#pragma unroll 8
      for (int q = 0; q < 64; ++q) sacc += red8[((q << 2) | (tid >> 3)) * 8 + (tid & 7)];
      a.dbpart[(long long)(sx * 4) * a.CDp + cd0 + tid] = sacc;
#pragma unroll
      for (int w2 = 1; w2 < 4; ++w2) a.dbpart[(long long)(sx * 4 + w2) * a.CDp + cd0 + tid] = 0.f;
    }
  }
}

template <bool GBF, bool DBF>
static int launch_wgrad_tr1_t(const WArgs& a, int S, hipStream_t s) {
  auto kern = wgrad_tr1_kernel<GBF, DBF>;
  dim3 grid(S, a.CGp / 32, a.CDp / 32);
  hipLaunchKernelGGL(kern, grid, dim3(256), 2 * 256 * 64 + 256, s, a);
  return launch_status("conv wgrad 1x1x1 bf16 (transposed reads)");
}

static int launch_wgrad_tr1(const WArgs& a, int S, hipStream_t s) {
  if (a.g_bf && a.d_bf) return launch_wgrad_tr1_t<true, true>(a, S, s);
  if (a.g_bf) return launch_wgrad_tr1_t<true, false>(a, S, s);
  if (a.d_bf) return launch_wgrad_tr1_t<false, true>(a, S, s);
  return launch_wgrad_tr1_t<false, false>(a, S, s);
}

#ifdef MMTTA_ACT_LEAKY_TU
constexpr bool WGRAD_RAW_KERNELS = false;
#else
constexpr bool WGRAD_RAW_KERNELS = true;
#endif
template <int TZ, int TY, int SI, bool TD, int NB>
static int launch_wgrad_tr_raw(const WArgs& a, int S, bool both, hipStream_t s) {
  if (both) return launch_wgrad_tr_t<TZ, TY, SI, true, true, TD, NB, true, true>(a, S, s);
  return launch_wgrad_tr_t<TZ, TY, SI, true, true, TD, NB, TD, !TD>(a, S, s);
}

template <int TZ, int TY, int SI>
static int launch_wgrad_tr(const WArgs& a, int S, hipStream_t s, int ncb = 1, int raw = 0) {
  MMTTA_CHECK(a.gvec4 && a.dvec4, MMTTA_ERR_INVALID, "wgrad: transposed-read kernel selected for unaligned tensors");
  MMTTA_CHECK(ncb == 1 || (a.g_bf && a.d_bf), MMTTA_ERR_INVALID, "wgrad: paired column blocks exist for the all-bf16 forms");
  if constexpr (WGRAD_RAW_KERNELS && SI == 2) {
    if ((raw & 2) && a.g_bf && a.d_bf) {
      const bool both = (raw & 1) != 0;
      if (a.convt) return ncb == 2 ? launch_wgrad_tr_raw<TZ, TY, SI, true, 2>(a, S, both, s) : launch_wgrad_tr_raw<TZ, TY, SI, true, 1>(a, S, both, s);
      return ncb == 2 ? launch_wgrad_tr_raw<TZ, TY, SI, false, 2>(a, S, both, s) : launch_wgrad_tr_raw<TZ, TY, SI, false, 1>(a, S, both, s);
    }
  }
  if (ncb == 2) {
    if constexpr (SI == 2) {
      if (a.convt) return launch_wgrad_tr_t<TZ, TY, SI, true, true, true, 2>(a, S, s);
    }
    MMTTA_CHECK(!a.convt, MMTTA_ERR_UNSUPPORTED, "wgrad: conv_transpose is stride 2 only");
    return launch_wgrad_tr_t<TZ, TY, SI, true, true, false, 2>(a, S, s);
  }
  if (a.convt) {
    MMTTA_CHECK(!a.g_bf || a.d_bf, MMTTA_ERR_UNSUPPORTED, "wgrad: a bf16-stored gradient needs a bf16-stored module input");
    if constexpr (SI == 2) {
      if (a.g_bf) return launch_wgrad_tr_t<TZ, TY, SI, true, true, true>(a, S, s);
      if (a.d_bf) return launch_wgrad_tr_t<TZ, TY, SI, false, true, true>(a, S, s);
      return launch_wgrad_tr_t<TZ, TY, SI, false, false, true>(a, S, s);
    }
    return MMTTA_ERR_UNSUPPORTED;
  }
  MMTTA_CHECK(!a.d_bf || a.g_bf, MMTTA_ERR_UNSUPPORTED, "wgrad: a bf16-stored gradient needs a bf16-stored module input");
  if (a.d_bf) return launch_wgrad_tr_t<TZ, TY, SI, true, true, false>(a, S, s);
  if (a.g_bf) return launch_wgrad_tr_t<TZ, TY, SI, true, false, false>(a, S, s);
  return launch_wgrad_tr_t<TZ, TY, SI, false, false, false>(a, S, s);
}

#ifdef MMTTA_ACT_LEAKY_TU
constexpr bool WGRAD_UPD_KERNELS = false;
#else
constexpr bool WGRAD_UPD_KERNELS = true;
#endif
template <int TZ, int TY, int SI, bool TD, int NB, bool RG, bool RD>
static int launch_wgrad_tr_upd_t(const WArgs& a, const UpdArgs& u, const PSets& ps, int kind, int S, hipStream_t s) {
  using G = WTGeo<TZ, TY, SI>;
  static_assert(G::lds_bytes(NB) >= (int)((UPD_CD * UPD_RS + 2) * sizeof(float)), "the update tile and its two scalars fit the images");
  static constexpr void (*kinds[3])(WArgs, UpdArgs, PSets) = {
      wgrad_tr_upd_kernel<TZ, TY, SI, TD, NB, RG, RD, MMTTA_OPTIM_ADAM>, wgrad_tr_upd_kernel<TZ, TY, SI, TD, NB, RG, RD, MMTTA_OPTIM_ADAMW>,
      wgrad_tr_upd_kernel<TZ, TY, SI, TD, NB, RG, RD, MMTTA_OPTIM_SGD>};
  static bool attr_set = false;
  if (!attr_set) {
    for (int k = 0; k < 3; ++k) (void)hipFuncSetAttribute((const void*)kinds[k], hipFuncAttributeMaxDynamicSharedMemorySize, 160 * 1024);
    attr_set = true;
  }
  dim3 grid(S, a.CGp / 32, a.CDp / 32 / NB);
  hipLaunchKernelGGL(kinds[kind], grid, dim3(256), G::lds_bytes(NB), s, a, u, ps);
  return launch_status("conv wgrad bf16 (transposed reads, update in the epilogue)");
}

template <int TZ, int TY>
static int launch_wgrad_tr_upd_s1(const WArgs& a, const UpdArgs& u, const PSets& ps, int kind, int S, hipStream_t s) {
  if constexpr (WGRAD_UPD_KERNELS) return launch_wgrad_tr_upd_t<TZ, TY, 1, false, 1, false, false>(a, u, ps, kind, S, s);
  set_error("wgrad: no kernel updates in its epilogue in this translation unit");
  return MMTTA_ERR_UNSUPPORTED;
}

struct W2Args {
  const float* q; long long qsn, qsd, qsh, qsw; int Cs, Dq, Hq, Wq; NL tq;
  const float* p; long long psn, psd, psh, psw; int Cb, Dp, Hp, Wp; NL tp;
  int si, ntaps;
  float* slab;
  float* dbpart;
  int tz, ty, tx, tiles, tiles_per_split, CBp;
  int S, tiles_set;
  int qvec4, pvec4;
  int p_bf;
  int p_thin;
  int q_bf;
  int bf;
};

template <bool PBF, int SI, bool T27>
__global__ __launch_bounds__(256) void wgrad_small_kernel(W2Args a) {
  extern __shared__ float lds[];
  constexpr int TZ = 4, TY = 4, TX = 8, MT = 128;
  const int tid = threadIdx.x, lane = tid & 63;
  const int wave = __builtin_amdgcn_readfirstlane(tid >> 6);
  const int h = lane >> 5, r = lane & 31;
  constexpr int NT = T27 ? 27 : 1;
  constexpr int ext = T27 ? 2 : 0;
  constexpr int BZ = (TZ - 1) * SI + ext + 1, BY = (TY - 1) * SI + ext + 1, BX = (TX - 1) * SI + ext + 1;
  constexpr int boxvox = BZ * BY * BX;
  constexpr int dmin = T27 ? -1 : 0;
  float* ql = lds;
  float* pl = lds + boxvox * 4;
  const int cb0 = blockIdx.y * 32;
  const int nrows = NT * a.Cs;
  const int rowid = wave * 32 + r;
  int toffl = 0;
  if (rowid < nrows) {
    const int tap = rowid / a.Cs, cs = rowid % a.Cs;
    toffl = (!T27 ? 0 : (((tap / 9) * BY + ((tap / 3) % 3)) * BX + (tap % 3))) * 4 + cs;
  }
  f32x16 acc;
#pragma unroll
  for (int i = 0; i < 16; ++i) acc[i] = 0.f;
  float dbacc = 0.f;
  const int sx = (int)xcd_contiguous_id(blockIdx.x, gridDim.x);
  const int qset = sx / a.S, sls = sx - qset * a.S;
  const int t0 = qset * a.tiles_set + sls * a.tiles_per_split;
  const int t1 = min((qset + 1) * a.tiles_set, t0 + a.tiles_per_split);
  const int tpn = a.tz * a.ty * a.tx;
  constexpr int NQ = (boxvox + 255) / 256;
  const bool piped = a.qvec4 && a.pvec4;
  float4 raw[NQ], praw[MT / 32];
  float qsc[4], qsh[4], psc[4], psh[4];
  const int pcv = tid & 7, pc = cb0 + pcv * 4;
  const int pcl4 = min(pc, (a.Cb - 1) & ~3);
  int n_coef = -1;
  auto decode = [&](int tile, int& n, int& oz0, int& oy0, int& ox0) {
    n = tile / tpn;
    int t = tile % tpn;
    const int txi = t % a.tx; t /= a.tx;
    const int tyi = t % a.ty;
    const int tzi = t / a.ty;
    oz0 = tzi * TZ; oy0 = tyi * TY; ox0 = txi * TX;
  };
  auto issue = [&](int tile) {
    int n, oz0, oy0, ox0;
    decode(tile, n, oz0, oy0, ox0);
    const int iz0 = oz0 * SI + dmin, iy0 = oy0 * SI + dmin, ix0 = ox0 * SI + dmin;
    const float* qb = a.q + (long long)n * a.qsn;
#pragma unroll
    for (int q = 0; q < NQ; ++q) {
      const int bv = min(tid + 256 * q, boxvox - 1);
      const int bx = bv % BX, by = (bv / BX) % BY, bz = bv / (BX * BY);
      const int iz = min(max(iz0 + bz, 0), a.Dq - 1), iy = min(max(iy0 + by, 0), a.Hq - 1), ix = min(max(ix0 + bx, 0), a.Wq - 1);
      raw[q] = *reinterpret_cast<const float4*>(qb + iz * a.qsd + iy * a.qsh + ix * a.qsw);
    }
    const long long pbo = (long long)n * a.psn;
#pragma unroll
    for (int q = 0; q < MT / 32; ++q) {
      const int v = (tid >> 3) + 32 * q;
      const int xl = v % TX, yl = (v / TX) % TY, zl = v / (TX * TY);
      const int oz = min(oz0 + zl, a.Dp - 1), oy = min(oy0 + yl, a.Hp - 1), ox = min(ox0 + xl, a.Wp - 1);
      praw[q] = ld4_t<PBF>(a.p, pbo + (long long)oz * a.psd + (long long)oy * a.psh + (long long)ox * a.psw + pcl4);
    }
    if (n != n_coef) {
      nl_coeff_vec<4>(a.tq, n, a.Cs, 0, qsc, qsh);
      nl_coeff_vec<4>(a.tp, n, a.Cb, pc, psc, psh);
      n_coef = n;
    }
  };
  auto commit = [&](int tile) {
    int n, oz0, oy0, ox0;
    decode(tile, n, oz0, oy0, ox0);
    const int iz0 = oz0 * SI + dmin, iy0 = oy0 * SI + dmin, ix0 = ox0 * SI + dmin;
#pragma unroll
    for (int q = 0; q < NQ; ++q) {
      const int bv = tid + 256 * q;
      if (bv < boxvox) {
        const int bx = bv % BX, by = (bv / BX) % BY, bz = bv / (BX * BY);
        const int iz = iz0 + bz, iy = iy0 + by, ix = ix0 + bx;
        float4 v = make_float4(0.f, 0.f, 0.f, 0.f);
        if ((unsigned)iz < (unsigned)a.Dq && (unsigned)iy < (unsigned)a.Hq && (unsigned)ix < (unsigned)a.Wq) {
          v.x = nl_apply(raw[q].x, qsc[0], qsh[0], a.tq.relu);
          v.y = a.Cs > 1 ? nl_apply(raw[q].y, qsc[1], qsh[1], a.tq.relu) : 0.f;
          v.z = a.Cs > 2 ? nl_apply(raw[q].z, qsc[2], qsh[2], a.tq.relu) : 0.f;
          v.w = a.Cs > 3 ? nl_apply(raw[q].w, qsc[3], qsh[3], a.tq.relu) : 0.f;
        }
        *reinterpret_cast<float4*>(ql + bv * 4) = v;
      }
    }
#pragma unroll
    for (int q = 0; q < MT / 32; ++q) {
      const int v = (tid >> 3) + 32 * q;
      const int xl = v % TX, yl = (v / TX) % TY, zl = v / (TX * TY);
      const int oz = oz0 + zl, oy = oy0 + yl, ox = ox0 + xl;
      float4 o = make_float4(0.f, 0.f, 0.f, 0.f);
      if (oz < a.Dp && oy < a.Hp && ox < a.Wp && pc < a.Cb) {
        const float4 x4 = praw[q];
        o.x = nl_apply(x4.x, psc[0], psh[0], a.tp.relu);
        o.y = (pc + 1 < a.Cb) ? nl_apply(x4.y, psc[1], psh[1], a.tp.relu) : 0.f;
        o.z = (pc + 2 < a.Cb) ? nl_apply(x4.z, psc[2], psh[2], a.tp.relu) : 0.f;
        o.w = (pc + 3 < a.Cb) ? nl_apply(x4.w, psc[3], psh[3], a.tp.relu) : 0.f;
      }
      *reinterpret_cast<float4*>(pl + v * 32 + pcv * 4) = o;
    }
  };
  if (piped && t0 < t1) issue(t0);
  for (int tile = t0; tile < t1; ++tile) {
    if (piped) {
      commit(tile);
    } else {
    const int n = tile / tpn;
    int t = tile % tpn;
    const int txi = t % a.tx; t /= a.tx;
    const int tyi = t % a.ty;
    const int tzi = t / a.ty;
    const int oz0 = tzi * TZ, oy0 = tyi * TY, ox0 = txi * TX;
    const int iz0 = oz0 * SI + dmin, iy0 = oy0 * SI + dmin, ix0 = ox0 * SI + dmin;
    {
      const float* qb = a.q + (long long)n * a.qsn;
      float sc[4], sh[4];
      nl_coeff_vec<4>(a.tq, n, a.Cs, 0, sc, sh);
      if (a.qvec4) {
#pragma unroll
        for (int q = 0; q < NQ; ++q) {
          const int bv = min(tid + 256 * q, boxvox - 1);
          const int bx = bv % BX, by = (bv / BX) % BY, bz = bv / (BX * BY);
          const int iz = min(max(iz0 + bz, 0), a.Dq - 1), iy = min(max(iy0 + by, 0), a.Hq - 1), ix = min(max(ix0 + bx, 0), a.Wq - 1);
          raw[q] = *reinterpret_cast<const float4*>(qb + iz * a.qsd + iy * a.qsh + ix * a.qsw);
        }
      } else {
// ... 675 lines not shown
  else if (tr) { TZ = 2; TY = 4; }
  w.tz = (w.dn->d + TZ - 1) / TZ;
  w.ty = (w.dn->h + TY - 1) / TY;
  w.tx = (w.dn->w + 7) / 8;
  w.tiles = w.tz * w.ty * w.tx * w.ips;
  w.CGp = roundup(w.g->c, 32);
  w.CDp = roundup(w.dn->c, 32);
  if (tr && g_wgrad_pair && (w.si == 2 || w.CDp <= 128 || g_wgrad_pair >= 2) && is_bf16(w.g) && is_bf16(w.dn) && (w.CDp / 32) % 2 == 0)
    w.ncb = 2;
  const int blocks_cc = (w.CGp / 32) * (w.CDp / 32 / w.ncb);
  int S = g_tune[2] / blocks_cc;
  if (tr1) S = 1024 / blocks_cc;
  plan_slabs(w, S, (int64_t)w.ntaps * w.CGp * w.CDp, w.ntaps == 1 ? 4 : 1);
  plan_bias(w, w.convt ? WB_COLSUMS : WB_MAIN_PARTIALS, dy);
  return MMTTA_OK;
}

template <int TZ, int TY, int TX, int NTW, bool GBF, bool DBF>
static int launch_wgrad_t(const WArgs& a, int S, hipStream_t s) {
  const int ext = a.ntaps == 1 ? 0 : 2;
  const int BZ = (TZ - 1) * a.si + ext + 1, BY = (TY - 1) * a.si + ext + 1, BX = (TX - 1) * a.si + ext + 1;
  const size_t lds = ((size_t)BZ * BY * BX + TZ * TY * TX) * 32 * sizeof(float);
  auto kern = wgrad_f32_kernel<TZ, TY, TX, NTW, GBF, DBF>;
  static bool attr_set = false;
  if (!attr_set) {
    (void)hipFuncSetAttribute((const void*)kern, hipFuncAttributeMaxDynamicSharedMemorySize, 160 * 1024);
    attr_set = true;
  }
  dim3 grid(S, a.CGp / 32, a.CDp / 32);
  hipLaunchKernelGGL(kern, grid, dim3(256), lds, s, a);
  return launch_status("conv wgrad");
}

template <int TZ, int TY, int TX, int NTW>
static int launch_wgrad(const WArgs& a, int S, hipStream_t s) {
  static constexpr int (*by_storage[2][2])(const WArgs&, int, hipStream_t) = {
      {launch_wgrad_t<TZ, TY, TX, NTW, false, false>, launch_wgrad_t<TZ, TY, TX, NTW, false, true>},
      {launch_wgrad_t<TZ, TY, TX, NTW, true, false>, launch_wgrad_t<TZ, TY, TX, NTW, true, true>}};
  return by_storage[a.g_bf][a.d_bf](a, S, s);
}

static int check_update_target(const mmtta_conv_desc* d, const WGeo& w, const mmtta_update_target* upd, UpdArgs& ua) {
  MMTTA_CHECK(route_reduce27(w.route), MMTTA_ERR_UNSUPPORTED,
              "wgrad update: the layer's weight gradient does not end in the 27-tap reduction");
  MMTTA_CHECK(upd->w_p && upd->w_m && upd->step && upd->image[0] && (upd->optim.kind == MMTTA_OPTIM_SGD || upd->w_v),
              MMTTA_ERR_INVALID, "wgrad update: null weight, moment, image or step pointer");
  MMTTA_CHECK(upd->b_p == nullptr || (!w.convt && upd->b_m && (upd->optim.kind == MMTTA_OPTIM_SGD || upd->b_v)),
              MMTTA_ERR_UNSUPPORTED, "wgrad update: the bias is updated here for Conv3d only (ConvTranspose3d: b_grad)");
  MMTTA_CHECK(upd->optim.kind >= MMTTA_OPTIM_ADAM && upd->optim.kind <= MMTTA_OPTIM_SGD, MMTTA_ERR_INVALID,
              "wgrad update: optimizer kind %d", upd->optim.kind);
  const mmtta_optim_desc& o = upd->optim;
  MMTTA_CHECK(!(o.kind == MMTTA_OPTIM_SGD && o.nesterov && (o.momentum <= 0.f || o.dampening != 0.f)), MMTTA_ERR_INVALID,
              "wgrad update: nesterov needs momentum > 0 and zero dampening");
  ua.a = OptimArgs{o.lr, o.beta1, o.beta2, o.eps, o.weight_decay, o.momentum, o.dampening, o.nesterov};
  ua.wp = upd->w_p; ua.wm = upd->w_m; ua.wv = upd->w_v;
  ua.bp = upd->b_p; ua.bm = upd->b_m; ua.bv = upd->b_v;
  ua.step = upd->step; ua.w_decay = upd->w_decay ? 1 : 0; ua.b_decay = upd->b_decay ? 1 : 0;
  for (int m = 0; m < 2; ++m) {
    ua.img[m].p = (unsigned short*)upd->image[m];
    ua.img[m].outer = upd->image_outer[m]; ua.img[m].inner = upd->image_inner[m];
    ua.img[m].Kp = ua.img[m].Np = ua.img[m].kn_is_ba = 0;
    if (upd->image[m] == nullptr) continue;
    mmtta_conv_desc dd = *d;
    if (m == 1) dd.op = w.convt ? MMTTA_CONVT_DGRAD : MMTTA_CONV_DGRAD;
    PackImageGeo g;
    const int st = pack_image_geometry(&dd, g);
    if (st) return st;
    MMTTA_CHECK(g.plain_bf16 && g.T == 27, MMTTA_ERR_UNSUPPORTED, "wgrad update: image %d is not a 27-tap bf16 image", m);
    MMTTA_CHECK(g.A == w.dn->c && g.B == w.g->c, MMTTA_ERR_INVALID, "wgrad update: image %d does not match the gradient", m);
    MMTTA_CHECK(((uintptr_t)upd->image[m]) % 16 == 0 && upd->image_outer[m] % 16 == 0 && upd->image_inner[m] % 16 == 0,
                MMTTA_ERR_INVALID, "wgrad update: images must keep 16-byte alignment");
    ua.img[m].Kp = g.Kp; ua.img[m].Np = g.Np; ua.img[m].kn_is_ba = g.kn_is_ba;
  }
  return MMTTA_OK;
}

static int launch_tiny_family(const mmtta_conv_desc* d, const WGeo& w, const mmtta_tensor* x, const mmtta_norm_on_load* x_norm,
                              const mmtta_tensor* dy, float* ws, float* dbws, hipStream_t s) {
  MMTTA_CHECK(is_f32(x) && is_f32(dy), MMTTA_ERR_UNSUPPORTED, "wgrad (tiny layer): fp32-stored tensors only");
  WTArgs t;
  t.x = tv(x); t.tx = nl(x_norm); t.dy = tv(dy);
  t.part = ws; t.ld = 27 * d->cin * d->cout;
  t.dbpart = dbws;
  t.B = w.tiny_blocks; t.ips = w.ips; t.BT = w.tiny_blocks * w.nsets;
  if (t.tx.mean != nullptr || t.tx.scale != nullptr) launch_tiny<true>(t, d->cin, d->cout, t.BT, s);
  else launch_tiny<false>(t, d->cin, d->cout, t.BT, s);
  return launch_status("wgrad tiny");
}

static int launch_thin_family(const mmtta_conv_desc* d, const WGeo& w, const mmtta_norm_on_load* x_norm, float* ws, float* dbws,
                              hipStream_t s) {
  const int Q = w.nsets;
  const bool thin_tr = w.route == W_THIN_TR;
  W2Args b;
  b.q = (const float*)w.q->ptr; b.qsn = w.q->sn; b.qsd = w.q->sd; b.qsh = w.q->sh; b.qsw = w.q->sw;
  b.Cs = w.q->c; b.Dq = w.q->d; b.Hq = w.q->h; b.Wq = w.q->w;
  b.p = (const float*)w.pb->ptr; b.psn = w.pb->sn; b.psd = w.pb->sd; b.psh = w.pb->sh; b.psw = w.pb->sw;
  b.Cb = w.pb->c; b.Dp = w.pb->d; b.Hp = w.pb->h; b.Wp = w.pb->w;
  b.tq = w.q_is_x ? nl(x_norm) : nl(nullptr);
  b.tp = w.q_is_x ? nl(nullptr) : nl(x_norm);
  b.si = w.si; b.ntaps = w.ntaps;
  b.slab = ws;
  b.dbpart = dbws;
  b.tz = w.tz; b.ty = w.ty; b.tx = w.tx; b.tiles = w.tiles * Q; b.tiles_per_split = w.tps; b.CBp = w.CDp;
  b.S = w.S; b.tiles_set = w.tiles;
  b.qvec4 = quad_aligned(w.q, 16) ? 1 : 0;
  b.pvec4 = quad_aligned(w.pb, quad_bytes(w.pb)) ? 1 : 0;
  MMTTA_CHECK(is_f32(w.q) || thin_tr, MMTTA_ERR_UNSUPPORTED, "wgrad (thin layer): the <= 4-channel tensor must be fp32-stored");
  b.p_bf = is_bf16(w.pb) ? 1 : 0;
  b.bf = (d->dtype == MMTTA_BF16 && w.ntaps == 27) ? 1 : 0;
  b.p_thin = w.p_thin ? 1 : 0;
  b.q_bf = is_bf16(w.q) ? 1 : 0;
  MMTTA_CHECK(!b.q_bf || thin_tr, MMTTA_ERR_UNSUPPORTED, "wgrad (thin layer): a bf16-stored <= 4-channel tensor needs the transposed-read kernel");
  const int ext = w.ntaps == 1 ? 0 : 2;
  const int BZ = 3 * w.si + ext + 1, BY = 3 * w.si + ext + 1, BX = 7 * w.si + ext + 1;
  const size_t lds = ((size_t)BZ * BY * BX * 4 + 128 * 32) * sizeof(float);
  MMTTA_CHECK((w.ntaps == 27 && (w.si == 1 || w.si == 2)) || (w.ntaps == 1 && w.si == 1), MMTTA_ERR_UNSUPPORTED,
              "wgrad (thin layer): %d taps with stride %d", w.ntaps, w.si);
  if (thin_tr) {
    launch_thin_tr(b, w.si, w.ncb, dim3(w.S * Q, w.CDp / 32 / w.ncb), s);
  } else {
    static constexpr decltype(&wgrad_small_kernel<false, 1, false>) forms[2][3] = {
        {wgrad_small_kernel<false, 1, false>, wgrad_small_kernel<false, 1, true>, wgrad_small_kernel<false, 2, true>},
        {wgrad_small_kernel<true, 1, false>, wgrad_small_kernel<true, 1, true>, wgrad_small_kernel<true, 2, true>}};
    const auto kern = forms[b.p_bf][w.ntaps == 1 ? 0 : w.si];
    hipLaunchKernelGGL(kern, dim3(w.S * Q, w.CDp / 32), dim3(256), lds, s, b);
  }
  return launch_status("wgrad small");
}

static int wgrad_raw_bits(const WGeo& w, const mmtta_norm_on_load* x_norm) {
  if (!WGRAD_RAW_KERNELS || !(g_raw_staging & 2) || w.route != W_TR_S2) return 0;
  const mmtta_tensor *xin = w.convt ? w.dn : w.g, *grad = w.convt ? w.g : w.dn;
  if (!is_bf16(xin) || !is_bf16(grad) || grad->c % 8 != 0) return 0;
  const bool ident = x_norm == nullptr || (x_norm->mean == nullptr && x_norm->scale == nullptr && x_norm->relu == MMTTA_ACT_NONE);
  return 2 | ((ident && xin->c % 8 == 0) ? 1 : 0);
}

static bool wgrad_updates_in_epilogue(const WGeo& w) {
  if (!WGRAD_UPD_KERNELS || !g_wgrad_epilogue_update) return false;
  if (w.route != W_TR_S1 || w.convt || w.ncb != 1) return false;
  if (w.nsl != 1 || w.pre_chunks != 0) return false;
  if (!is_bf16(w.g) || !is_bf16(w.dn)) return false;
  return w.g->c % 32 == 0 && w.dn->c % 32 == 0;
}
static bool update_target_vec16(const mmtta_update_target* upd, const PSets& ps, int nsets) {
  const bool keep_m = upd->optim.kind != MMTTA_OPTIM_SGD || upd->optim.momentum != 0.f;
  auto al = [](const void* p) { return p != nullptr && ((uintptr_t)p & 15) == 0; };
  if (!al(upd->w_p) || (keep_m && !al(upd->w_m)) || (upd->optim.kind != MMTTA_OPTIM_SGD && !al(upd->w_v))) return false;
  if (nsets > 1 && (ps.weight_outer % 4 != 0 || (ps.inner != 1 && ps.weight_inner % 4 != 0))) return false;
  return true;
}

static int launch_main_family(const WGeo& w, const mmtta_tensor* x, const mmtta_norm_on_load* x_norm, float* ws, float* dbws,
                              hipStream_t s, const UpdArgs* ua = nullptr, const PSets* ps = nullptr, int kind = 0) {
  WArgs a;
  a.g = (const float*)w.g->ptr; a.gsn = w.g->sn; a.gsd = w.g->sd; a.gsh = w.g->sh; a.gsw = w.g->sw;
  a.Cg = w.g->c; a.Dgg = w.g->d; a.Hgg = w.g->h; a.Wgg = w.g->w;
  a.dn = (const float*)w.dn->ptr; a.dsn = w.dn->sn; a.dsd = w.dn->sd; a.dsh = w.dn->sh; a.dsw = w.dn->sw;
  a.Cd = w.dn->c; a.Dd = w.dn->d; a.Hd = w.dn->h; a.Wd = w.dn->w;
  a.tg = w.convt ? nl(nullptr) : nl(x_norm);
  a.td = w.convt ? nl(x_norm) : nl(nullptr);
  a.N = x->n;
  a.si = w.si; a.ntaps = w.ntaps;
  a.slab = ws;
  a.dbpart = dbws;
  a.tz = w.tz; a.ty = w.ty; a.tx = w.tx; a.tiles = w.tiles * w.nsets; a.tiles_per_split = w.tps;
  a.S = w.S; a.tiles_set = w.tiles;
  a.CGp = w.CGp; a.CDp = w.CDp;
  a.g_bf = is_bf16(w.g) ? 1 : 0;
  a.d_bf = is_bf16(w.dn) ? 1 : 0;
  a.convt = w.convt ? 1 : 0;
  a.gvec4 = quad_aligned(w.g, quad_bytes(w.g)) ? 1 : 0;
  a.dvec4 = quad_aligned(w.dn, quad_bytes(w.dn)) ? 1 : 0;
  const int SQ = w.S * w.nsets;
  if (ua != nullptr) return launch_wgrad_tr_upd_s1<4, 8>(a, *ua, *ps, kind, SQ, s);
  switch (w.route) {
    case W_TR_1X1: return launch_wgrad_tr1(a, SQ, s);
    case W_TR_S1: return launch_wgrad_tr<4, 8, 1>(a, SQ, s, w.ncb, wgrad_raw_bits(w, x_norm));
    case W_TR_S2: return launch_wgrad_tr<2, 4, 2>(a, SQ, s, w.ncb, wgrad_raw_bits(w, x_norm));
    case W_F32_1X1: return launch_wgrad<4, 4, 8, 1>(a, SQ, s);
    case W_F32_S1: return launch_wgrad<4, 4, 8, 7>(a, SQ, s);
    default: return launch_wgrad<2, 2, 8, 7>(a, SQ, s);
  }
}

static int reduce_tail(const WGeo& w, const mmtta_tensor* dy, float* ws, float* dw, float* db, int accumulate,
                       const mmtta_param_sets* sets, const mmtta_update_target* upd, const UpdArgs& ua, bool updated, hipStream_t s) {
  const PSets ps = psets(sets);
  const int Q = w.nsets;
  const bool tiny = w.route == W_TINY, thin = route_thin(w.route);
  float* dbws = ws + w.slab_floats * Q;
  const float* rsrc = ws;
  int rn = w.nsl, st;
  if (w.pre_chunks > 0) {
    float* pre = ws + (w.slab_floats + w.db_floats) * Q;
    const long long elems = w.slab_elems;
    hipLaunchKernelGGL(slab_prereduce_kernel, dim3((unsigned)((elems + 255) / 256), w.pre_chunks, Q), dim3(256), 0, s, ws, pre,
                       w.nsl, elems);
    st = launch_status(thin ? "wgrad small prereduce" : "wgrad prereduce");
    if (st) return st;
    rsrc = pre; rn = w.pre_chunks;
  }
  const bool db_rides = db != nullptr && w.bias == WB_MAIN_PARTIALS && route_reduce27(w.route);
  const int Cg = thin ? w.q->c : w.g->c, Cd = thin ? w.pb->c : w.dn->c;
  switch (w.route) {
    case W_TINY: {
      const int ld = 27 * Cg * Cd;
      hipLaunchKernelGGL(db_reduce_kernel, dim3(ld, Q), dim3(64), 0, s, rsrc, dw, w.tiny_blocks, ld, ld, accumulate, ps, 1);
      break;
    }
    case W_SMALL:
    case W_THIN_TR:
      hipLaunchKernelGGL(wgrad_small_reduce_kernel, dim3((w.ntaps * Cg * Cd + 255) / 256, Q), dim3(256), 0, s, rsrc, dw, rn, w.ntaps,
                         Cg, Cd, w.CDp, w.small_is_cd, accumulate, ps);
      break;
    case W_F32_1X1:
    case W_TR_1X1:
      hipLaunchKernelGGL(wgrad_reduce1_kernel, dim3((Cg + 31) / 32, (Cd + 31) / 32, Q), dim3(256), 0, s, rsrc, dw, rn,
                         Cg, Cd, w.CGp, w.CDp, accumulate, ps);
      break;
    default:
      if (updated) break;
      if (upd != nullptr) {
        static constexpr decltype(&wgrad_update27_kernel<0>) kinds[3] = {
            wgrad_update27_kernel<MMTTA_OPTIM_ADAM>, wgrad_update27_kernel<MMTTA_OPTIM_ADAMW>, wgrad_update27_kernel<MMTTA_OPTIM_SGD>};
        const auto kern = kinds[upd->optim.kind];
        hipLaunchKernelGGL(kern, dim3((Cg + UPD_CG - 1) / UPD_CG + (db_rides ? 1 : 0), (Cd + UPD_CD - 1) / UPD_CD, Q),
                           dim3(256), 0, s, rsrc, rn, Cg, Cd, w.CGp, w.CDp, dbws, w.nsl, ps, ua);
      } else {
        hipLaunchKernelGGL(wgrad_reduce27_kernel, dim3(Cg + (db_rides ? 1 : 0), (Cd + 31) / 32, Q), dim3(256), 0, s, rsrc, dw, rn,
                           Cg, Cd, w.CGp, w.CDp, accumulate, dbws, db_rides ? db : nullptr, w.nsl, ps);
      }
  }
  st = launch_status(tiny ? "wgrad tiny reduce" : thin ? "wgrad small reduce" : upd != nullptr ? "wgrad update" : "wgrad reduce");
  if (st || db == nullptr || db_rides) return st;
  int rows = w.nsl, ld = w.CDp;
  if (w.bias == WB_TINY_PARTIALS) { rows = w.tiny_blocks; ld = 4; }
  if (w.bias == WB_COLSUMS) {
    st = launch_channel_sums(dy, dbws, s);
    if (st) return st;
    rows = (int)w.colsum_blocks; ld = 2 * dy->c;
  }
  hipLaunchKernelGGL(db_reduce_kernel, dim3(dy->c, Q), dim3(64), 0, s, dbws, db, rows, dy->c, ld, accumulate, ps, 0);
  return launch_status(tiny ? "wgrad tiny reduce" : "bias reduce");
}

int conv_wgrad_body(const mmtta_conv_desc* d, const mmtta_tensor* x, const mmtta_norm_on_load* x_norm,
                    const mmtta_tensor* dy, float* dw, float* db, int accumulate, void* workspace,
                    int64_t workspace_bytes, const mmtta_param_sets* sets, void* stream, const mmtta_update_target* upd) {
  WGeo w{};
  int st = wgeometry(d, x, dy, sets, w);
  if (st) return st;
  UpdArgs ua;
  if (upd != nullptr) {
    st = check_update_target(d, w, upd, ua);
    if (st) return st;
    dw = upd->w_p;
    db = w.convt ? upd->b_grad : upd->b_p;
  }
  MMTTA_CHECK(dw != nullptr, MMTTA_ERR_INVALID, "wgrad: null dw");
  const int64_t need = (w.slab_floats + w.db_floats + w.pre_floats) * w.nsets * 4;
  MMTTA_CHECK(workspace != nullptr && workspace_bytes >= need, MMTTA_ERR_WORKSPACE, "wgrad: workspace %lld bytes, need %lld",
              (long long)workspace_bytes, (long long)need);
  hipStream_t s = (hipStream_t)stream;
  float* ws = (float*)workspace;
  const PSets ps = psets(sets);
  const bool in_epilogue = upd != nullptr && wgrad_updates_in_epilogue(w) && update_target_vec16(upd, ps, w.nsets);
  float* dbws = (db != nullptr && w.bias != WB_COLSUMS) ? ws + w.slab_floats * w.nsets : nullptr;
  if (w.route == W_TINY) st = launch_tiny_family(d, w, x, x_norm, dy, ws, dbws, s);
  else if (route_thin(w.route)) st = launch_thin_family(d, w, x_norm, ws, dbws, s);
  else if (in_epilogue) st = launch_main_family(w, x, x_norm, ws, dbws, s, &ua, &ps, upd->optim.kind);
  else st = launch_main_family(w, x, x_norm, ws, dbws, s);
  if (st || (g_profile_main_only && upd == nullptr)) return st;
  return reduce_tail(w, dy, ws, dw, db, accumulate, sets, upd, ua, in_epilogue, s);
}

MMTTA_ACT_NS_CLOSE
}

#ifndef MMTTA_ACT_LEAKY_TU
using namespace mmtta;

extern "C" int64_t mmtta_conv_wgrad_workspace_bytes_sets(const mmtta_conv_desc* d, const mmtta_tensor* x, const mmtta_tensor* dy,
                                                         const mmtta_param_sets* sets) {
  WGeo w{};
  if (wgeometry(d, x, dy, sets, w)) return -1;
  return (w.slab_floats + w.db_floats + w.pre_floats) * w.nsets * (int64_t)sizeof(float);
}

extern "C" int64_t mmtta_conv_wgrad_workspace_bytes(const mmtta_conv_desc* d, const mmtta_tensor* x,
                                                    const mmtta_tensor* dy) {
  return mmtta_conv_wgrad_workspace_bytes_sets(d, x, dy, nullptr);
}

extern "C" int mmtta_conv_wgrad_plan_sets(const mmtta_conv_desc* d, const mmtta_tensor* x, const mmtta_tensor* dy,
                                          const mmtta_param_sets* sets, int32_t plan[4]) {
  MMTTA_CHECK(plan != nullptr, MMTTA_ERR_INVALID, "wgrad plan: null output");
  WGeo w{};
  const int st = wgeometry(d, x, dy, sets, w);
  if (st) return st;
  plan[0] = w.nsl; plan[1] = w.pre_chunks; plan[2] = w.CGp; plan[3] = w.CDp;
  return MMTTA_OK;
}

extern "C" int mmtta_conv_wgrad_kernel(const mmtta_conv_desc* d, const mmtta_tensor* x, const mmtta_tensor* dy) {
  WGeo w{};
  const int st = wgeometry(d, x, dy, nullptr, w);
  if (st) return st < 0 ? st : -st;
  return w.route;
}

extern "C" int mmtta_conv_wgrad_stages_raw(const mmtta_conv_desc* d, const mmtta_tensor* x, const mmtta_norm_on_load* x_norm,
                                           const mmtta_tensor* dy) {
  WGeo w{};
  const int st = wgeometry(d, x, dy, nullptr, w);
  if (st) return st < 0 ? st : -st;
  return nl_leaky(x_norm) ? 0 : wgrad_raw_bits(w, x_norm);
}

extern "C" int mmtta_conv_wgrad(const mmtta_conv_desc* d, const mmtta_tensor* x, const mmtta_norm_on_load* x_norm,
                                const mmtta_tensor* dy, float* dw, float* db, int accumulate, void* workspace,
                                int64_t workspace_bytes, void* stream) {
  return mmtta_conv_wgrad_sets(d, x, x_norm, dy, dw, db, accumulate, workspace, workspace_bytes, nullptr, stream);
}

extern "C" int mmtta_conv_wgrad_sets(const mmtta_conv_desc* d, const mmtta_tensor* x, const mmtta_norm_on_load* x_norm,
                                     const mmtta_tensor* dy, float* dw, float* db, int accumulate, void* workspace,
                                     int64_t workspace_bytes, const mmtta_param_sets* sets, void* stream) {
  {
    int st = nl_act_check(x_norm, "conv_wgrad (x_norm)");
    if (st) return st;
    st = nl_per_item_check(x_norm, "conv_wgrad (x_norm)");
    if (st) return st;
  }
  if (nl_leaky(x_norm))
    return leaky::conv_wgrad_body(d, x, x_norm, dy, dw, db, accumulate, workspace, workspace_bytes, sets, stream, nullptr);
  return conv_wgrad_body(d, x, x_norm, dy, dw, db, accumulate, workspace, workspace_bytes, sets, stream, nullptr);
}

extern "C" int mmtta_conv_wgrad_updates_in_epilogue(const mmtta_conv_desc* d, const mmtta_tensor* x, const mmtta_norm_on_load* x_norm,
                                                    const mmtta_tensor* dy, const mmtta_param_sets* sets) {
  WGeo w{};
  const int st = wgeometry(d, x, dy, sets, w);
  if (st) return st < 0 ? st : -st;
  if (g_fused_update == 0 || !route_reduce27(w.route)) return 0;
  return (!nl_leaky(x_norm) && wgrad_updates_in_epilogue(w)) ? 1 : 0;
}

extern "C" int mmtta_fused_update_enabled(void) { return g_fused_update != 0 ? 1 : 0; }

extern "C" int mmtta_conv_wgrad_update_sets(const mmtta_conv_desc* d, const mmtta_tensor* x, const mmtta_norm_on_load* x_norm,
                                            const mmtta_tensor* dy, const mmtta_update_target* target, void* workspace,
                                            int64_t workspace_bytes, const mmtta_param_sets* sets, void* stream) {
  MMTTA_CHECK(g_fused_update != 0, MMTTA_ERR_UNSUPPORTED, "wgrad update: switched off (MMTTA_FUSED_UPDATE=0)");
  MMTTA_CHECK(target != nullptr, MMTTA_ERR_INVALID, "wgrad update: null target");
  {
    int st = nl_act_check(x_norm, "conv_wgrad_update (x_norm)");
    if (st) return st;
    st = nl_per_item_check(x_norm, "conv_wgrad_update (x_norm)");
    if (st) return st;
  }
  if (nl_leaky(x_norm))
    return leaky::conv_wgrad_body(d, x, x_norm, dy, nullptr, nullptr, 0, workspace, workspace_bytes, sets, stream, target);
  return conv_wgrad_body(d, x, x_norm, dy, nullptr, nullptr, 0, workspace, workspace_bytes, sets, stream, target);
}
#endif
```

### multimodal_tta_amd/csrc/conv_wgrad_tr_body.h

```cpp
  using G = WTGeo<TZ, TY, SI>;
  static_assert(TY % 2 == 0, "a k step is two rows of one z slice");
  static_assert((!RG || GBF) && (!RD || DBF), "raw staging copies bf16-stored items");
  constexpr bool NEEDC = TD ? !RD : !RG;
  extern __shared__ float lds[];
  unsigned char* gl = reinterpret_cast<unsigned char*>(lds);
  unsigned char* dl = gl + G::G_BYTES;
  const int tid = threadIdx.x, lane = tid & 63;
  const int wave = __builtin_amdgcn_readfirstlane(tid >> 6);
  const int h = lane >> 5, r = lane & 31;
  const int cg0 = blockIdx.y * 32, cd0 = blockIdx.z * 32 * NB;

  const int lq = (lane & 15) >> 2, lp = lane & 3, lc = (lane >> 4) & 1;
  const unsigned char* dread = dl + (h * 8 + lq) * 64 + lc * 32 + lp * 8;
  const unsigned char* gread[7];
#pragma unroll
  for (int j = 0; j < 7; ++j) {
    const int tap = min(wave + 4 * j, 26);
    gread[j] = gl + (h * SI * G::BX + lq) * 64 + lc * 32 + lp * 8 + G::tap_off(tap);
  }
  f32x16 acc[NB][7];
#pragma unroll
  for (int nb = 0; nb < NB; ++nb)
#pragma unroll
    for (int j = 0; j < 7; ++j)
#pragma unroll
      for (int i = 0; i < 16; ++i) acc[nb][j][i] = 0.f;
  float dbs[NB][8];
#pragma unroll
  for (int nb = 0; nb < NB; ++nb)
#pragma unroll
    for (int c = 0; c < 8; ++c) dbs[nb][c] = 0.f;
  const bool want_db = a.dbpart != nullptr && blockIdx.y == 0;

  const int rsub = min(tid / G::IPR, G::RPP - 1);
  const int rem = tid % G::IPR, bx = rem >> 2, c8 = rem & 3;
  const int bxm = SI == 1 ? bx : (bx & 1) * G::XH + (bx >> 1);
  unsigned char* gst = gl + (rsub * G::BX + bxm) * 64 + c8 * 16;
  const int dvox0 = tid >> 2, d8 = tid & 3;
  unsigned char* dst = dl + dvox0 * 64 + d8 * 16;
  const int dzl = dvox0 / (TY * 8), dyl = (dvox0 >> 3) % TY, dxl = dvox0 & 7;
  const int gcb = cg0 + 8 * c8, dcb = cd0 + 8 * d8;
  const unsigned gc_lo = GBF ? min(gcb, (a.Cg - 1) & ~7) : min(gcb, (a.Cg - 1) & ~3), gc_hi = min(gcb + 4, (a.Cg - 1) & ~3);
  const unsigned dc_lo = DBF ? min(dcb, (a.Cd - 1) & ~7) : min(dcb, (a.Cd - 1) & ~3), dc_hi = min(dcb + 4, (a.Cd - 1) & ~3);
  const unsigned dc_lo1 = DBF ? min(dcb + 32, (a.Cd - 1) & ~7) : min(dcb + 32, (a.Cd - 1) & ~3), dc_hi1 = min(dcb + 36, (a.Cd - 1) & ~3);
  const bool gtail = (a.Cg & 7) != 0, dtail = (a.Cd & 7) != 0;
  auto pair_mask = [](int c, int C) { return (c < C ? 0xffffu : 0u) | (c + 1 < C ? 0xffff0000u : 0u); };
  const unsigned gsd = (unsigned)a.gsd, gsh = (unsigned)a.gsh, gsw = (unsigned)a.gsw;
  const unsigned dsd = (unsigned)a.dsd, dsh = (unsigned)a.dsh, dsw = (unsigned)a.dsw;

  const int sx = (int)xcd_contiguous_id(blockIdx.x, gridDim.x);
  const int qset = sx / a.S, sls = sx - qset * a.S;
  const int t0 = qset * a.tiles_set + sls * a.tiles_per_split;
  const int t1 = min((qset + 1) * a.tiles_set, t0 + a.tiles_per_split);
  const int tpn = a.tz * a.ty * a.tx;
  constexpr int GP = G::GP, DP = G::DP;
  constexpr int PREF = (GBF || DBF) ? 40 : 32;
  constexpr int PGmax = (PREF - NB * DP * (DBF ? 4 : 8)) / (GBF ? 4 : 8);
  constexpr int PG = PGmax < 0 ? 0 : (PGmax < GP ? PGmax : GP);
  Oct8<GBF> gv[GP];
  Oct8<DBF> dq[NB * DP];
  unsigned pok = 0u;
  unsigned dok = 0u;
  int pn = -1, poz0 = 0, poy0 = 0, pox0 = 0;
  int cn = -1;
  float* coefl = reinterpret_cast<float*>(dl + NB * G::D_BYTES);
  const float relu_lo = act_lo(TD ? a.td.relu : a.tg.relu);
  unsigned gxoff = 0u;
  bool gxok = false;

  auto tile_x = [&](int ix0) {
    const int ix = ix0 + bx;
    gxok = (unsigned)ix < (unsigned)a.Wgg;
    gxoff = __umul24((unsigned)min(max(ix, 0), a.Wgg - 1), gsw);
  };
  auto load_g = [&](auto pc, const float* gbase, int iz0, int iy0) {
    constexpr int P = decltype(pc)::value;
    constexpr int row0 = G::RPP * P, bz0 = row0 / G::BY, by0 = row0 % G::BY;
    constexpr bool can_wrap = by0 + G::RPP > G::BY;
    int by = by0 + rsub;
    bool wrap = false;
    if constexpr (can_wrap) {
      wrap = by >= G::BY;
      by = wrap ? by - G::BY : by;
    }
    const int izA = iz0 + bz0, izB = izA + 1;
    const unsigned zoA = __umul24((unsigned)min(max(izA, 0), a.Dgg - 1), gsd), zoB = __umul24((unsigned)min(max(izB, 0), a.Dgg - 1), gsd);
    const bool zkA = (unsigned)izA < (unsigned)a.Dgg, zkB = (unsigned)izB < (unsigned)a.Dgg;
    const unsigned zo = (can_wrap && wrap) ? zoB : zoA;
    const bool zk = (can_wrap && wrap) ? zkB : zkA;
    const int iy = iy0 + by;
    const bool ok = zk && gxok && (unsigned)iy < (unsigned)a.Hgg;
    pok |= (ok ? 1u : 0u) << P;
    const unsigned off = zo + __umul24((unsigned)min(max(iy, 0), a.Hgg - 1), gsh) + gxoff;
    gv[P] = oct8_ld<GBF>(gbase, off + gc_lo, off + gc_hi);
  };
  auto commit_g = [&](auto pc, const float (&sc)[8], const float (&sh)[8]) {
    constexpr int P = decltype(pc)::value;
    unsigned okm = ((pok >> P) & 1u) ? 0xffffffffu : 0u;
    uint4 pk;
    if constexpr (RG) {
      if constexpr (!TD) okm = gcb < a.Cg ? okm : 0u;
      pk = gv[P].q;
      pk.x &= okm; pk.y &= okm; pk.z &= okm; pk.w &= okm;
    } else {
    float v[8];
    oct8_f8(gv[P], v);
    if constexpr (!TD) {
#pragma unroll
      for (int j = 0; j < 8; ++j) v[j] = act_max(fmaf(v[j], sc[j], sh[j]), relu_lo);
    }
    pk.x = wpack2(v[0], v[1]) & okm; pk.y = wpack2(v[2], v[3]) & okm;
    pk.z = wpack2(v[4], v[5]) & okm; pk.w = wpack2(v[6], v[7]) & okm;
    }
    if (gtail) {
      pk.x &= pair_mask(gcb, a.Cg); pk.y &= pair_mask(gcb + 2, a.Cg); pk.z &= pair_mask(gcb + 4, a.Cg); pk.w &= pair_mask(gcb + 6, a.Cg);
    }
    *reinterpret_cast<uint4*>(gst + P * (G::RPP * G::BX * 64)) = pk;
  };
  auto issue = [&](int tile) {
    pn = tile / tpn;
    int t = tile % tpn;
    const int txi = t % a.tx; t /= a.tx;
    const int tyi = t % a.ty;
    const int tzi = t / a.ty;
    poz0 = tzi * TZ; poy0 = tyi * TY; pox0 = txi * 8;
    const float* dbase = reinterpret_cast<const float*>(reinterpret_cast<const char*>(a.dn) + (long long)pn * a.dsn * (DBF ? 2 : 4));
    const int oy = poy0 + dyl, ox = pox0 + dxl;
    const bool yxok = oy < a.Hd && ox < a.Wd;
    const unsigned yxoff = __umul24((unsigned)min(oy, a.Hd - 1), dsh) + __umul24((unsigned)min(ox, a.Wd - 1), dsw);
    dok = 0u;
#pragma unroll
    for (int p = 0; p < DP; ++p) {
      const int oz = poz0 + dzl + p * (64 / (TY * 8));
      dok |= ((yxok && oz < a.Dd) ? 1u : 0u) << p;
      const unsigned off = __umul24((unsigned)min(oz, a.Dd - 1), dsd) + yxoff;
      dq[p] = oct8_ld<DBF>(dbase, off + dc_lo, off + dc_hi);
      if constexpr (NB == 2) dq[DP + p] = oct8_ld<DBF>(dbase, off + dc_lo1, off + dc_hi1);
    }
    pok = 0u;
    tile_x(pox0 * SI - 1);
    const float* gbase = reinterpret_cast<const float*>(reinterpret_cast<const char*>(a.g) + (long long)pn * a.gsn * (GBF ? 2 : 4));
    static_for<0, PG>([&](auto pc) { load_g(pc, gbase, poz0 * SI - 1, poy0 * SI - 1); });
  };

  if (t0 < t1) issue(t0);
  for (int tile = t0; tile < t1; ++tile) {
    const int n = pn;
    constexpr int RB = GBF ? 12 : 4;
    constexpr int R1 = PG + RB < GP ? PG + RB : GP;
    const float* gbase = reinterpret_cast<const float*>(reinterpret_cast<const char*>(a.g) + (long long)n * a.gsn * (GBF ? 2 : 4));
    const int iz0 = poz0 * SI - 1, iy0 = poy0 * SI - 1;
    static_for<PG, R1>([&](auto pc) { load_g(pc, gbase, iz0, iy0); });
    if (NEEDC && n != cn) {
      if constexpr (NB == 1) {
        float s8[8], h8[8];
        if constexpr (TD) nl_coeff_vec<8>(a.td, n, a.Cd, dcb, s8, h8);
        else nl_coeff_vec<8>(a.tg, n, a.Cg, gcb, s8, h8);
        const int k8 = TD ? d8 : c8;
#pragma unroll
        for (int j = 0; j < 8; ++j) { coefl[8 * k8 + j] = s8[j]; coefl[32 + 8 * k8 + j] = h8[j]; }
      } else {
#pragma unroll
      for (int nb = 0; nb < (TD ? NB : 1); ++nb) {
        float s8[8], h8[8];
        if constexpr (TD) nl_coeff_vec<8>(a.td, n, a.Cd, dcb + 32 * nb, s8, h8);
        else nl_coeff_vec<8>(a.tg, n, a.Cg, gcb, s8, h8);
        const int k8 = TD ? d8 : c8;
#pragma unroll
        for (int j = 0; j < 8; ++j) { coefl[64 * nb + 8 * k8 + j] = s8[j]; coefl[64 * nb + 32 + 8 * k8 + j] = h8[j]; }
      }
      }
      cn = n;
      __syncthreads();
    }
    float sc[8], sh[8];
    if constexpr (NB == 1) {
    if constexpr (NEEDC) {
      const float4* cq = reinterpret_cast<const float4*>(coefl + 8 * (TD ? d8 : c8));
      const float4 s0 = cq[0], s1 = cq[1], h0 = cq[8], h1 = cq[9];
      sc[0] = s0.x; sc[1] = s0.y; sc[2] = s0.z; sc[3] = s0.w; sc[4] = s1.x; sc[5] = s1.y; sc[6] = s1.z; sc[7] = s1.w;
      sh[0] = h0.x; sh[1] = h0.y; sh[2] = h0.z; sh[3] = h0.w; sh[4] = h1.x; sh[5] = h1.y; sh[6] = h1.z; sh[7] = h1.w;
    }
#pragma unroll
    for (int p = 0; p < DP; ++p) {
      float v[8];
      if constexpr (!RD) oct8_f8(dq[p], v);
      if constexpr (TD && !RD) {
#pragma unroll
        for (int j = 0; j < 8; ++j) v[j] = act_max(fmaf(v[j], sc[j], sh[j]), relu_lo);
      }
      const unsigned okm = ((dok >> p) & 1u) ? 0xffffffffu : 0u;
      if (want_db) {
        if constexpr (RD) oct8_f8(dq[p], v);
#pragma unroll
        for (int j = 0; j < 8; ++j) {
          const unsigned cm = (dcb + j < a.Cd) ? okm : 0u;
          dbs[0][j] += __uint_as_float(__float_as_uint(v[j]) & cm);
        }
      }
      uint4 pk;
      if constexpr (RD) {
        const unsigned dm = (!TD || dcb < a.Cd) ? okm : 0u;
        pk = dq[p].q;
        pk.x &= dm; pk.y &= dm; pk.z &= dm; pk.w &= dm;
      } else {
      pk.x = wpack2(v[0], v[1]) & okm; pk.y = wpack2(v[2], v[3]) & okm;
      pk.z = wpack2(v[4], v[5]) & okm; pk.w = wpack2(v[6], v[7]) & okm;
      }
      if (dtail) {
        pk.x &= pair_mask(dcb, a.Cd); pk.y &= pair_mask(dcb + 2, a.Cd); pk.z &= pair_mask(dcb + 4, a.Cd); pk.w &= pair_mask(dcb + 6, a.Cd);
      }
      *reinterpret_cast<uint4*>(dst + p * 4096) = pk;
    }
    } else {
#define MMTTA_COEF_REGS(nb)                                                                                            \
    {                                                                                                                  \
      const float4* cq = reinterpret_cast<const float4*>(coefl + 64 * (nb) + 8 * (TD ? d8 : c8));                      \
      const float4 s0 = cq[0], s1 = cq[1], h0 = cq[8], h1 = cq[9];                                                     \
      sc[0] = s0.x; sc[1] = s0.y; sc[2] = s0.z; sc[3] = s0.w; sc[4] = s1.x; sc[5] = s1.y; sc[6] = s1.z; sc[7] = s1.w; \
      sh[0] = h0.x; sh[1] = h0.y; sh[2] = h0.z; sh[3] = h0.w; sh[4] = h1.x; sh[5] = h1.y; sh[6] = h1.z; sh[7] = h1.w; \
    }
    if constexpr (NEEDC && (!TD || NB == 1)) MMTTA_COEF_REGS(0)
#pragma unroll
    for (int nb = 0; nb < NB; ++nb) {
    if constexpr (NEEDC && TD && NB > 1) MMTTA_COEF_REGS(nb)
    const int dcn = dcb + 32 * nb;
#pragma unroll
    for (int p = 0; p < DP; ++p) {
      float v[8];
      if constexpr (!RD) oct8_f8(dq[nb * DP + p], v);
      if constexpr (TD && !RD) {
#pragma unroll
        for (int j = 0; j < 8; ++j) v[j] = act_max(fmaf(v[j], sc[j], sh[j]), relu_lo);
      }
      const unsigned okm = ((dok >> p) & 1u) ? 0xffffffffu : 0u;
      if (want_db) {
        if constexpr (RD) oct8_f8(dq[nb * DP + p], v);
#pragma unroll
        for (int j = 0; j < 8; ++j) {
          const unsigned cm = (dcn + j < a.Cd) ? okm : 0u;
          dbs[nb][j] += __uint_as_float(__float_as_uint(v[j]) & cm);
        }
      }
      uint4 pk;
      if constexpr (RD) {
        const unsigned dm = (!TD || dcn < a.Cd) ? okm : 0u;
        pk = dq[nb * DP + p].q;
        pk.x &= dm; pk.y &= dm; pk.z &= dm; pk.w &= dm;
      } else {
      pk.x = wpack2(v[0], v[1]) & okm; pk.y = wpack2(v[2], v[3]) & okm;
      pk.z = wpack2(v[4], v[5]) & okm; pk.w = wpack2(v[6], v[7]) & okm;
      }
      if (dtail) {
        pk.x &= pair_mask(dcn, a.Cd); pk.y &= pair_mask(dcn + 2, a.Cd); pk.z &= pair_mask(dcn + 4, a.Cd); pk.w &= pair_mask(dcn + 6, a.Cd);
      }
      *reinterpret_cast<uint4*>(dst + nb * G::D_BYTES + p * 4096) = pk;
    }
    }
    }
    static_for<0, R1>([&](auto pc) { commit_g(pc, sc, sh); });
    if constexpr (R1 < GP) {
      constexpr int R2 = R1 + RB < GP ? R1 + RB : GP;
      static_for<R1, R2>([&](auto pc) { load_g(pc, gbase, iz0, iy0); });
      static_for<R1, R2>([&](auto pc) { commit_g(pc, sc, sh); });
      if constexpr (R2 < GP) {
        static_for<R2, GP>([&](auto pc) { load_g(pc, gbase, iz0, iy0); });
        static_for<R2, GP>([&](auto pc) { commit_g(pc, sc, sh); });
      }
    }
    __syncthreads();
    if (tile + 1 < t1) issue(tile + 1);
    constexpr int LA = 3, NF = G::NK * 7;
    wbf16x8 ra[LA + 1], fb[2][NB];
#pragma unroll
    for (int nb = 0; nb < NB; ++nb) fb[0][nb] = MMTTA_TR_FRAG(dread, nb * G::D_BYTES);
#pragma unroll
    for (int f = 0; f < LA; ++f) ra[f] = MMTTA_TR_FRAG(gread[f % 7], G::row_off(f / 7));
    __builtin_amdgcn_sched_barrier(0);
#pragma unroll
    for (int f = 0; f < NF; ++f) {
      const int ks = f / 7, j = f % 7;
      if (f + LA < NF) ra[(f + LA) % (LA + 1)] = MMTTA_TR_FRAG(gread[(f + LA) % 7], G::row_off((f + LA) / 7));
      if (j == 2 && ks + 1 < G::NK) {
#pragma unroll
        for (int nb = 0; nb < NB; ++nb) fb[(ks + 1) & 1][nb] = MMTTA_TR_FRAG(dread, nb * G::D_BYTES + (ks + 1) * 1024);
      }
#pragma unroll
      for (int nb = 0; nb < NB; ++nb)
        acc[nb][j] = __builtin_amdgcn_mfma_f32_32x32x16_bf16(ra[f % (LA + 1)], fb[ks & 1][nb], acc[nb][j], 0, 0, 0);
      __builtin_amdgcn_sched_barrier(0);
    }
    __syncthreads();
  }
  if constexpr (UPD) {
    float* tile = lds;
    float* scal = lds + UPD_CD * UPD_RS;
    const int t0s = *u.step;
    if (tid == 0) optim_scalars(KIND, u.a, t0s, scal[0], scal[1]);
    const bool first = t0s == 0;
    const bool wd_on = u.a.wd != 0.f;
    const bool keep_m = KIND != 2 || u.a.momentum != 0.f;
    __syncthreads();
    const float step_size = scal[0], bc2_sqrt = scal[1];
    if (want_db) {
      float* red8 = lds;
#pragma unroll
      for (int nb = 0; nb < NB; ++nb) {
        if (nb) __syncthreads();
#pragma unroll
        for (int c = 0; c < 8; ++c) red8[tid * 8 + c] = dbs[nb][c];
        __syncthreads();
        const int cd = cd0 + 32 * nb + tid;
        if (tid < 32 && cd < a.Cd) {
          float sacc = 0.f;
#pragma unroll 8
          for (int q = 0; q < 64; ++q) sacc += red8[((q << 2) | (tid >> 3)) * 8 + (tid & 7)];
          const float t = 0.f + sacc;
          const long long o = pset_bias_elems(ps, qset) + cd;
          float pi = u.bp[o], mi = 0.f, vi = 0.f;
          if (!first) {
            if (keep_m) mi = u.bm[o];
            if (KIND != 2) vi = u.bv[o];
          }
          optim_update<KIND>(pi, t, mi, vi, wd_on && u.b_decay, u.a, step_size, bc2_sqrt, first);
          u.bp[o] = pi;
          if (keep_m) u.bm[o] = mi;
          if (KIND != 2) u.bv[o] = vi;
        }
      }
      __syncthreads();
    }
    const bool decay = wd_on && u.w_decay;
    const long long wo = pset_weight_elems(ps, qset), rowst = (long long)a.Cg * 27;
#pragma unroll
    for (int nb = 0; nb < NB; ++nb)
#pragma unroll
    for (int g = 0; g < 4; ++g) {
#pragma unroll
      for (int j = 0; j < 7; ++j) {
        const int tap = wave + 4 * j;
        if (tap < 27) {
#pragma unroll
          for (int i = 0; i < 4; ++i) tile[r * UPD_RS + (i + 4 * h) * 27 + tap] = 0.f + acc[nb][j][4 * g + i];
        }
      }
      __syncthreads();
      const int ucg0 = cg0 + 8 * g, ucd0 = cd0 + 32 * nb;
      const long long ob = wo + ((long long)ucd0 * a.Cg + ucg0) * 27;
      upd_optim4<KIND, 4>(u, ob, rowst, 0, ucd0, a.Cd, first, keep_m, decay, step_size, bc2_sqrt, tile);
      upd_optim4<KIND, 3>(u, ob, rowst, 4, ucd0, a.Cd, first, keep_m, decay, step_size, bc2_sqrt, tile);
      __syncthreads();
#pragma unroll
      for (int m = 0; m < 2; ++m) upd_repack(u.img[m], ps, qset, ucg0, ucd0, tile);
      __syncthreads();
    }
  } else {
  const int sl = sx;
#pragma unroll
  for (int nb = 0; nb < NB; ++nb)
#pragma unroll
  for (int j = 0; j < 7; ++j) {
    const int tap = wave + 4 * j;
    if (tap < 27) {
      float* sb = a.slab + (((long long)sl * 27 + tap) * a.CGp + cg0) * a.CDp + cd0 + 32 * nb + r;
#pragma unroll
      for (int i = 0; i < 16; ++i) {
        const int row = (i & 3) + 8 * (i >> 2) + 4 * h;
        sb[(long long)row * a.CDp] = acc[nb][j][i];
      }
    }
  }
  if (want_db) {
    float* red8 = lds;
#pragma unroll
    for (int nb = 0; nb < NB; ++nb) {
      if (nb) __syncthreads();
#pragma unroll
      for (int c = 0; c < 8; ++c) red8[tid * 8 + c] = dbs[nb][c];
      __syncthreads();
      if (tid < 32) {
        float sacc = 0.f;
#pragma unroll 8
        for (int q = 0; q < 64; ++q) sacc += red8[((q << 2) | (tid >> 3)) * 8 + (tid & 7)];
        a.dbpart[(long long)sl * a.CDp + cd0 + 32 * nb + tid] = sacc;
      }
    }
  }
  }
```

Baseline: 125.5.

## Load wgrad dense operand directly to LDS with double-buffered global_load_lds

Adds a stride-1 bf16 wgrad kernel variant, plus a fused-update variant, that moves the dense (dy) tile straight into LDS with global_load_lds into a double-buffered image. This replaces the register staging, convert and write path. Loads for the next tile are issued before the MFMA loop and waited on afterwards, and the bias gradient is read back from LDS. It is gated by an option that is on by default and by shape and alignment checks. LDS use doubles for the dense operand and more register budget goes to prefetching the other operand, which may lower occupancy.

New measurement: 126.1 (median of 6 runs). About the same (+0.5%).

```diff
diff --git a/include/mmtta.h b/include/mmtta.h
--- a/include/mmtta.h
+++ b/include/mmtta.h
@@ -67,6 +67,7 @@
 #define MMTTA_OPT_WGRAD_EPILOGUE_UPDATE 19
 #define MMTTA_OPT_CLS8_PIPELINE 20
 #define MMTTA_OPT_CLS8_LEAN_EPILOGUE 21
+#define MMTTA_OPT_WGRAD_DENSE_DMA 22
 int mmtta_set_option(int key, int value);
 
 int mmtta_copy_strided(const mmtta_tensor* src, const mmtta_tensor* dst, void* stream);
@@ -449,6 +450,8 @@
                                  int64_t workspace_bytes, const mmtta_param_sets* sets, void* stream);
 int mmtta_conv_wgrad_updates_in_epilogue(const mmtta_conv_desc* desc, const mmtta_tensor* x, const mmtta_norm_on_load* x_norm,
                                          const mmtta_tensor* dy, const mmtta_param_sets* sets);
+int mmtta_conv_wgrad_dense_dma(const mmtta_conv_desc* desc, const mmtta_tensor* x, const mmtta_norm_on_load* x_norm,
+                               const mmtta_tensor* dy, const mmtta_param_sets* sets, int fused_update);
 
 int mmtta_optim_step_segments(const mmtta_optim_desc* desc, float* p, const float* g, float* m, float* v, const int64_t* segments,
                               int count, int64_t total, int sets, int64_t set_stride, int32_t* step, void* stream);
diff --git a/multimodal_tta_amd/_lib.py b/multimodal_tta_amd/_lib.py
--- a/multimodal_tta_amd/_lib.py
+++ b/multimodal_tta_amd/_lib.py
@@ -268,6 +268,7 @@
     "mmtta_conv_wgrad_update_sets": (C.c_int, [_P(ConvDesc), _P(Tensor), _P(NormOnLoad), _P(Tensor), _P(UpdateTarget),
                                                C.c_void_p, C.c_int64, _P(ParamSets), C.c_void_p]),
     "mmtta_conv_wgrad_updates_in_epilogue": (C.c_int, [_P(ConvDesc), _P(Tensor), _P(NormOnLoad), _P(Tensor), _P(ParamSets)]),
+    "mmtta_conv_wgrad_dense_dma": (C.c_int, [_P(ConvDesc), _P(Tensor), _P(NormOnLoad), _P(Tensor), _P(ParamSets), C.c_int]),
     "mmtta_sam_ascent_partials": (C.c_int64, [C.c_int64, C.c_int]),
     "mmtta_sam_ascent_sets": (C.c_int, [C.c_void_p, C.c_void_p, C.c_void_p, C.c_int64, C.c_void_p, C.c_int64, C.c_int, C.c_int,
                                         C.c_int64, C.c_float, C.c_void_p]),
@@ -345,6 +346,8 @@
         lib.mmtta_set_option(20, int(os.environ["MMTTA_CLS8PIPE"]))
     if "MMTTA_CLS8LEAN" in os.environ:
         lib.mmtta_set_option(21, int(os.environ["MMTTA_CLS8LEAN"]))
+    if "MMTTA_DENSEDMA" in os.environ:
+        lib.mmtta_set_option(22, int(os.environ["MMTTA_DENSEDMA"]))
     _lib = lib
     return lib
 
diff --git a/multimodal_tta_amd/csrc/api.hip b/multimodal_tta_amd/csrc/api.hip
--- a/multimodal_tta_amd/csrc/api.hip
+++ b/multimodal_tta_amd/csrc/api.hip
@@ -24,6 +24,7 @@
 int g_wgrad_epilogue_update = 1;
 int g_cls8_pipeline = 1;
 int g_cls8_lean_epilogue = 1;
+int g_wgrad_dense_dma = 1;
 int g_tune[4] = {96, 128, 128, 256};
 }
 
@@ -98,6 +99,11 @@
     mmtta::g_cls8_lean_epilogue = value & 1;
     return prev;
   }
+  if (key == MMTTA_OPT_WGRAD_DENSE_DMA) {
+    const int prev = mmtta::g_wgrad_dense_dma;
+    mmtta::g_wgrad_dense_dma = value & 1;
+    return prev;
+  }
   if (key == MMTTA_OPT_IGEMM_PIPELINE) {
     const int prev = mmtta::g_igemm_pipeline;
     mmtta::g_igemm_pipeline = value ? 1 : 0;
diff --git a/multimodal_tta_amd/csrc/common.h b/multimodal_tta_amd/csrc/common.h
--- a/multimodal_tta_amd/csrc/common.h
+++ b/multimodal_tta_amd/csrc/common.h
@@ -43,6 +43,7 @@
 extern int g_thin_lean;
 extern int g_wgrad_epilogue_update;
 extern int g_cls8_pipeline;
+extern int g_wgrad_dense_dma;
 extern int g_cls8_lean_epilogue;
 extern int g_tune[4];
 
diff --git a/multimodal_tta_amd/csrc/conv_wgrad.hip b/multimodal_tta_amd/csrc/conv_wgrad.hip
--- a/multimodal_tta_amd/csrc/conv_wgrad.hip
+++ b/multimodal_tta_amd/csrc/conv_wgrad.hip
@@ -606,6 +606,7 @@
   static constexpr int G_BYTES = NG * 64, D_BYTES = ND * 64;
   static constexpr int LDS_BYTES = G_BYTES + D_BYTES + 256;
   __host__ __device__ static constexpr int lds_bytes(int nb) { return G_BYTES + nb * (D_BYTES + 256); }
+  __host__ __device__ static constexpr int lds_bytes_dma(int nb) { return G_BYTES + nb * (2 * D_BYTES + 256); }
   static constexpr int NK = ND / 16;
   static constexpr int IPR = BX * 4;
   static constexpr int RPP = 256 / IPR;
@@ -625,11 +626,14 @@
 typedef short wshort4 __attribute__((ext_vector_type(4)));
 typedef short wshort8 __attribute__((ext_vector_type(8)));
 typedef __attribute__((address_space(3))) wshort4* wlds4_t;
+typedef unsigned wu32x4 __attribute__((ext_vector_type(4)));
 
 #define MMTTA_TR_FRAG(ptr, off)                                                                          \
   __builtin_bit_cast(wbf16x8, __builtin_shufflevector(__builtin_amdgcn_ds_read_tr16_b64_v4i16((wlds4_t)((ptr) + (off))),       \
                                                       __builtin_amdgcn_ds_read_tr16_b64_v4i16((wlds4_t)((ptr) + (off) + 256)), \
                                                       0, 1, 2, 3, 4, 5, 6, 7))
+
+__device__ __forceinline__ wbf16x8 wtr_frag_scoped(const unsigned char* __restrict__ p, int off) { return MMTTA_TR_FRAG(p, off); }
 
 #define MMTTA_TR_NO_UPDATE    \
   constexpr bool UPD = false; \
@@ -638,21 +642,33 @@
   constexpr PSets ps{};
 template <int TZ, int TY, int SI, bool GBF, bool DBF, bool TD, int NB = 1>
 __global__ __launch_bounds__(256, (NB == 1 && SI == 1) ? 2 : 1) void wgrad_tr_kernel(WArgs a) {
-  constexpr bool RG = false, RD = false;
+  constexpr bool RG = false, RD = false, DMA = false;
   MMTTA_TR_NO_UPDATE
 #include "conv_wgrad_tr_body.h"
 }
 
 template <int TZ, int TY, int SI, bool TD, int NB, bool RG, bool RD>
 __global__ __launch_bounds__(256, (NB == 1 && SI == 1) ? 2 : 1) void wgrad_tr_raw_kernel(WArgs a) {
-  constexpr bool GBF = true, DBF = true;
+  constexpr bool GBF = true, DBF = true, DMA = false;
   MMTTA_TR_NO_UPDATE
 #include "conv_wgrad_tr_body.h"
 }
 
 template <int TZ, int TY, int SI, bool TD, int NB, bool RG, bool RD, int KIND>
 __global__ __launch_bounds__(256, (NB == 1 && SI == 1) ? 2 : 1) void wgrad_tr_upd_kernel(WArgs a, UpdArgs u, PSets ps) {
-  constexpr bool GBF = true, DBF = true, UPD = true;
+  constexpr bool GBF = true, DBF = true, UPD = true, DMA = false;
+#include "conv_wgrad_tr_body.h"
+}
+
+template <int TZ, int TY, int SI, int NB>
+__global__ __launch_bounds__(256, (NB == 1 && SI == 1) ? 2 : 1) void wgrad_tr_dma_kernel(WArgs a) {
+  constexpr bool GBF = true, DBF = true, TD = false, RG = false, RD = false, DMA = true;
+  MMTTA_TR_NO_UPDATE
+#include "conv_wgrad_tr_body.h"
+}
+template <int TZ, int TY, int SI, int NB, int KIND>
+__global__ __launch_bounds__(256, (NB == 1 && SI == 1) ? 2 : 1) void wgrad_tr_upd_dma_kernel(WArgs a, UpdArgs u, PSets ps) {
+  constexpr bool GBF = true, DBF = true, TD = false, RG = false, RD = false, UPD = true, DMA = true;
 #include "conv_wgrad_tr_body.h"
 }
 
@@ -671,6 +687,34 @@
   dim3 grid(S, a.CGp / 32, a.CDp / 32 / NB);
   hipLaunchKernelGGL(kern, grid, dim3(256), G::lds_bytes(NB), s, a);
   return launch_status("conv wgrad bf16 (transposed reads)");
+}
+
+#ifdef MMTTA_ACT_LEAKY_TU
+constexpr bool WGRAD_DMA_KERNELS = false;
+#else
+constexpr bool WGRAD_DMA_KERNELS = true;
+#endif
+template <int TZ, int TY, int NB>
+static int launch_wgrad_tr_dma_t(const WArgs& a, int S, hipStream_t s) {
+  using G = WTGeo<TZ, TY, 1>;
+  auto kern = wgrad_tr_dma_kernel<TZ, TY, 1, NB>;
+  static bool attr_set = false;
+  if (!attr_set) {
+    (void)hipFuncSetAttribute((const void*)kern, hipFuncAttributeMaxDynamicSharedMemorySize, 160 * 1024);
+    attr_set = true;
+  }
+  MMTTA_CHECK((a.CDp / 32) % NB == 0, MMTTA_ERR_INVALID, "wgrad: %d dense column blocks in groups of %d", a.CDp / 32, NB);
+  dim3 grid(S, a.CGp / 32, a.CDp / 32 / NB);
+  hipLaunchKernelGGL(kern, grid, dim3(256), G::lds_bytes_dma(NB), s, a);
+  return launch_status("conv wgrad bf16 (transposed reads, dense operand by direct-to-LDS loads)");
+}
+template <int TZ, int TY>
+static int launch_wgrad_tr_dma_s1(const WArgs& a, int S, hipStream_t s, int ncb) {
+  if constexpr (WGRAD_DMA_KERNELS) {
+    if (ncb == 2) return launch_wgrad_tr_dma_t<TZ, TY, 2>(a, S, s);
+  }
+  set_error("wgrad: no kernel loads its dense operand directly to LDS in this translation unit");
+  return MMTTA_ERR_UNSUPPORTED;
 }
 
 template <bool GBF, bool DBF>
@@ -902,8 +946,27 @@
   return launch_status("conv wgrad bf16 (transposed reads, update in the epilogue)");
 }
 
+template <int TZ, int TY, int NB>
+static int launch_wgrad_tr_upd_dma_t(const WArgs& a, const UpdArgs& u, const PSets& ps, int kind, int S, hipStream_t s) {
+  using G = WTGeo<TZ, TY, 1>;
+  static constexpr void (*kinds[3])(WArgs, UpdArgs, PSets) = {
+      wgrad_tr_upd_dma_kernel<TZ, TY, 1, NB, MMTTA_OPTIM_ADAM>, wgrad_tr_upd_dma_kernel<TZ, TY, 1, NB, MMTTA_OPTIM_ADAMW>,
+      wgrad_tr_upd_dma_kernel<TZ, TY, 1, NB, MMTTA_OPTIM_SGD>};
+  static bool attr_set = false;
+  if (!attr_set) {
+    for (int k = 0; k < 3; ++k) (void)hipFuncSetAttribute((const void*)kinds[k], hipFuncAttributeMaxDynamicSharedMemorySize, 160 * 1024);
+    attr_set = true;
+  }
+  dim3 grid(S, a.CGp / 32, a.CDp / 32 / NB);
+  hipLaunchKernelGGL(kinds[kind], grid, dim3(256), G::lds_bytes_dma(NB), s, a, u, ps);
+  return launch_status("conv wgrad bf16 (transposed reads, dense operand by direct-to-LDS loads, update in the epilogue)");
+}
+
 template <int TZ, int TY>
-static int launch_wgrad_tr_upd_s1(const WArgs& a, const UpdArgs& u, const PSets& ps, int kind, int S, hipStream_t s) {
+static int launch_wgrad_tr_upd_s1(const WArgs& a, const UpdArgs& u, const PSets& ps, int kind, int S, hipStream_t s, bool dma) {
+  if constexpr (WGRAD_UPD_KERNELS && WGRAD_DMA_KERNELS) {
+    if (dma) return launch_wgrad_tr_upd_dma_t<TZ, TY, 1>(a, u, ps, kind, S, s);
+  }
   if constexpr (WGRAD_UPD_KERNELS) return launch_wgrad_tr_upd_t<TZ, TY, 1, false, 1, false, false>(a, u, ps, kind, S, s);
   set_error("wgrad: no kernel updates in its epilogue in this translation unit");
   return MMTTA_ERR_UNSUPPORTED;
@@ -1885,6 +1948,18 @@
   return true;
 }
 
+static bool wgrad_dense_dma(const WGeo& w, bool in_epilogue) {
+  if (!WGRAD_DMA_KERNELS || !(g_wgrad_dense_dma & 1)) return false;
+  if (w.route != W_TR_S1 || w.convt) return false;
+  if (w.ncb == 1 && !in_epilogue) return false;
+  const mmtta_tensor* dy = w.dn;
+  if (!is_bf16(w.g) || !is_bf16(dy)) return false;
+  if (dy->c % (32 * w.ncb) != 0) return false;
+  if (dy->d % 4 != 0 || dy->h % 8 != 0 || dy->w % 8 != 0) return false;
+  if (((uintptr_t)dy->ptr & 15) != 0) return false;
+  return dy->sw % 8 == 0 && dy->sh % 8 == 0 && dy->sd % 8 == 0 && dy->sn % 8 == 0;
+}
+
 static int launch_main_family(const WGeo& w, const mmtta_tensor* x, const mmtta_norm_on_load* x_norm, float* ws, float* dbws,
                               hipStream_t s, const UpdArgs* ua = nullptr, const PSets* ps = nullptr, int kind = 0) {
   WArgs a;
@@ -1907,10 +1982,12 @@
   a.gvec4 = quad_aligned(w.g, quad_bytes(w.g)) ? 1 : 0;
   a.dvec4 = quad_aligned(w.dn, quad_bytes(w.dn)) ? 1 : 0;
   const int SQ = w.S * w.nsets;
-  if (ua != nullptr) return launch_wgrad_tr_upd_s1<4, 8>(a, *ua, *ps, kind, SQ, s);
+  if (ua != nullptr) return launch_wgrad_tr_upd_s1<4, 8>(a, *ua, *ps, kind, SQ, s, wgrad_dense_dma(w, true));
   switch (w.route) {
     case W_TR_1X1: return launch_wgrad_tr1(a, SQ, s);
-    case W_TR_S1: return launch_wgrad_tr<4, 8, 1>(a, SQ, s, w.ncb, wgrad_raw_bits(w, x_norm));
+    case W_TR_S1:
+      if (wgrad_dense_dma(w, false)) return launch_wgrad_tr_dma_s1<4, 8>(a, SQ, s, w.ncb);
+      return launch_wgrad_tr<4, 8, 1>(a, SQ, s, w.ncb, wgrad_raw_bits(w, x_norm));
     case W_TR_S2: return launch_wgrad_tr<2, 4, 2>(a, SQ, s, w.ncb, wgrad_raw_bits(w, x_norm));
     case W_F32_1X1: return launch_wgrad<4, 4, 8, 1>(a, SQ, s);
     case W_F32_S1: return launch_wgrad<4, 4, 8, 7>(a, SQ, s);
@@ -2052,6 +2129,15 @@
   return nl_leaky(x_norm) ? 0 : wgrad_raw_bits(w, x_norm);
 }
 
+extern "C" int mmtta_conv_wgrad_dense_dma(const mmtta_conv_desc* d, const mmtta_tensor* x, const mmtta_norm_on_load* x_norm,
+                                          const mmtta_tensor* dy, const mmtta_param_sets* sets, int fused_update) {
+  WGeo w{};
+  const int st = wgeometry(d, x, dy, sets, w);
+  if (st) return st < 0 ? st : -st;
+  const bool in_epilogue = fused_update && g_fused_update != 0 && route_reduce27(w.route) && wgrad_updates_in_epilogue(w);
+  return (!nl_leaky(x_norm) && wgrad_dense_dma(w, in_epilogue)) ? 1 : 0;
+}
+
 extern "C" int mmtta_conv_wgrad(const mmtta_conv_desc* d, const mmtta_tensor* x, const mmtta_norm_on_load* x_norm,
                                 const mmtta_tensor* dy, float* dw, float* db, int accumulate, void* workspace,
                                 int64_t workspace_bytes, void* stream) {
diff --git a/multimodal_tta_amd/csrc/conv_wgrad_tr_body.h b/multimodal_tta_amd/csrc/conv_wgrad_tr_body.h
--- a/multimodal_tta_amd/csrc/conv_wgrad_tr_body.h
+++ b/multimodal_tta_amd/csrc/conv_wgrad_tr_body.h
@@ -1,6 +1,7 @@
   using G = WTGeo<TZ, TY, SI>;
   static_assert(TY % 2 == 0, "a k step is two rows of one z slice");
   static_assert((!RG || GBF) && (!RD || DBF), "raw staging copies bf16-stored items");
+  static_assert(!DMA || (SI == 1 && GBF && DBF && !TD && !RG && !RD), "direct-to-LDS loads: the bf16-stored gradient of a stride-1 convolution");
   constexpr bool NEEDC = TD ? !RD : !RG;
   extern __shared__ float lds[];
   unsigned char* gl = reinterpret_cast<unsigned char*>(lds);
@@ -55,7 +56,7 @@
   const int tpn = a.tz * a.ty * a.tx;
   constexpr int GP = G::GP, DP = G::DP;
   constexpr int PREF = (GBF || DBF) ? 40 : 32;
-  constexpr int PGmax = (PREF - NB * DP * (DBF ? 4 : 8)) / (GBF ? 4 : 8);
+  constexpr int PGmax = DMA ? PREF / 4 : (PREF - NB * DP * (DBF ? 4 : 8)) / (GBF ? 4 : 8);
   constexpr int PG = PGmax < 0 ? 0 : (PGmax < GP ? PGmax : GP);
   Oct8<GBF> gv[GP];
   Oct8<DBF> dq[NB * DP];
@@ -63,7 +64,12 @@
   unsigned dok = 0u;
   int pn = -1, poz0 = 0, poy0 = 0, pox0 = 0;
   int cn = -1;
-  float* coefl = reinterpret_cast<float*>(dl + NB * G::D_BYTES);
+  float* coefl = reinterpret_cast<float*>(dl + (DMA ? 2 : 1) * NB * G::D_BYTES);
+  constexpr int DIMG = NB * G::D_BYTES;
+  int dimg = 0, dtgt = 0;
+  const unsigned char* dcur = dread;
+  unsigned dlane = 0u;
+  if constexpr (DMA) dlane = (__umul24((unsigned)dyl, dsh) + __umul24((unsigned)dxl, dsw) + 8u * d8) * 2u;
   const float relu_lo = act_lo(TD ? a.td.relu : a.tg.relu);
   unsigned gxoff = 0u;
   bool gxok = false;
@@ -94,6 +100,26 @@
     const unsigned off = zo + __umul24((unsigned)min(max(iy, 0), a.Hgg - 1), gsh) + gxoff;
     gv[P] = oct8_ld<GBF>(gbase, off + gc_lo, off + gc_hi);
   };
+  auto box_off = [&](auto pc, int rs, int iz0, int iy0) -> unsigned {
+    constexpr int P = decltype(pc)::value;
+    constexpr int row0 = G::RPP * P, bz0 = row0 / G::BY, by0 = row0 % G::BY;
+    constexpr bool can_wrap = by0 + G::RPP > G::BY;
+    int by = by0 + rs;
+    bool wrap = false;
+    if constexpr (can_wrap) {
+      wrap = by >= G::BY;
+      by = wrap ? by - G::BY : by;
+    }
+    const int izA = iz0 + bz0, izB = izA + 1;
+    const unsigned zoA = __umul24((unsigned)min(max(izA, 0), a.Dgg - 1), gsd), zoB = __umul24((unsigned)min(max(izB, 0), a.Dgg - 1), gsd);
+    const bool zkA = (unsigned)izA < (unsigned)a.Dgg, zkB = (unsigned)izB < (unsigned)a.Dgg;
+    const unsigned zo = (can_wrap && wrap) ? zoB : zoA;
+    const bool zk = (can_wrap && wrap) ? zkB : zkA;
+    const int iy = iy0 + by;
+    const bool ok = zk && gxok && (unsigned)iy < (unsigned)a.Hgg;
+    pok |= (ok ? 1u : 0u) << P;
+    return zo + __umul24((unsigned)min(max(iy, 0), a.Hgg - 1), gsh) + gxoff;
+  };
   auto commit_g = [&](auto pc, const float (&sc)[8], const float (&sh)[8]) {
     constexpr int P = decltype(pc)::value;
     unsigned okm = ((pok >> P) & 1u) ? 0xffffffffu : 0u;
@@ -124,6 +150,23 @@
     const int tyi = t % a.ty;
     const int tzi = t / a.ty;
     poz0 = tzi * TZ; poy0 = tyi * TY; pox0 = txi * 8;
+    if constexpr (DMA) {
+      static_assert(!DMA || 64 / (TY * 8) == 1, "pass p of the dense tile is z slice p");
+      const char* src = reinterpret_cast<const char*>(a.dn) +
+                        ((long long)pn * a.dsn + (long long)poz0 * a.dsd + (long long)poy0 * a.dsh + (long long)pox0 * a.dsw + cd0) * 2;
+      unsigned char* dimage = dl + dtgt + wave * 1024;
+      unsigned dln = dlane;
+      asm volatile("" : "+v"(dln));
+#pragma unroll
+      for (int p = 0; p < DP; ++p)
+#pragma unroll
+        for (int nb = 0; nb < NB; ++nb) {
+          const char* sp = src + (long long)p * a.dsd * 2 + nb * 64;
+          asm volatile("" : "+s"(sp));
+          __builtin_amdgcn_global_load_lds((const __attribute__((address_space(1))) void*)(sp + dln),
+                                           (__attribute__((address_space(3))) void*)(dimage + nb * G::D_BYTES + p * 4096), 16, 0, 0);
+        }
+    } else {
     const float* dbase = reinterpret_cast<const float*>(reinterpret_cast<const char*>(a.dn) + (long long)pn * a.dsn * (DBF ? 2 : 4));
     const int oy = poy0 + dyl, ox = pox0 + dxl;
     const bool yxok = oy < a.Hd && ox < a.Wd;
@@ -137,10 +180,21 @@
       dq[p] = oct8_ld<DBF>(dbase, off + dc_lo, off + dc_hi);
       if constexpr (NB == 2) dq[DP + p] = oct8_ld<DBF>(dbase, off + dc_lo1, off + dc_hi1);
     }
+    }
     pok = 0u;
     tile_x(pox0 * SI - 1);
     const float* gbase = reinterpret_cast<const float*>(reinterpret_cast<const char*>(a.g) + (long long)pn * a.gsn * (GBF ? 2 : 4));
+    if constexpr (DMA) {
+      unsigned goff[PG];
+      int rs = rsub;
+      asm volatile("" : "+v"(rs));
+      static_for<0, PG>([&](auto pc) { goff[decltype(pc)::value] = box_off(pc, rs, poz0 * SI - 1, poy0 * SI - 1); });
+      __builtin_amdgcn_sched_barrier(0);
+      static_for<0, PG>([&](auto pc) { gv[decltype(pc)::value] = oct8_ld<GBF>(gbase, goff[decltype(pc)::value] + gc_lo, 0u); });
+      __builtin_amdgcn_sched_barrier(0);
+    } else {
     static_for<0, PG>([&](auto pc) { load_g(pc, gbase, poz0 * SI - 1, poy0 * SI - 1); });
+    }
   };
 
   if (t0 < t1) issue(t0);
@@ -181,6 +235,7 @@
       sc[0] = s0.x; sc[1] = s0.y; sc[2] = s0.z; sc[3] = s0.w; sc[4] = s1.x; sc[5] = s1.y; sc[6] = s1.z; sc[7] = s1.w;
       sh[0] = h0.x; sh[1] = h0.y; sh[2] = h0.z; sh[3] = h0.w; sh[4] = h1.x; sh[5] = h1.y; sh[6] = h1.z; sh[7] = h1.w;
     }
+    if constexpr (!DMA) {
 #pragma unroll
     for (int p = 0; p < DP; ++p) {
       float v[8];
@@ -212,6 +267,7 @@
       }
       *reinterpret_cast<uint4*>(dst + p * 4096) = pk;
     }
+    }
     } else {
 #define MMTTA_COEF_REGS(nb)                                                                                            \
     {                                                                                                                  \
@@ -225,6 +281,7 @@
     for (int nb = 0; nb < NB; ++nb) {
     if constexpr (NEEDC && TD && NB > 1) MMTTA_COEF_REGS(nb)
     const int dcn = dcb + 32 * nb;
+    if constexpr (!DMA) {
 #pragma unroll
     for (int p = 0; p < DP; ++p) {
       float v[8];
@@ -258,7 +315,25 @@
     }
     }
     }
+    }
     static_for<0, R1>([&](auto pc) { commit_g(pc, sc, sh); });
+    if constexpr (DMA) {
+      if (want_db) {
+        asm volatile("s_waitcnt vmcnt(0)" ::: "memory");
+#pragma unroll
+        for (int nb = 0; nb < NB; ++nb)
+#pragma unroll
+          for (int p = 0; p < DP; ++p) {
+            const wu32x4 q = *reinterpret_cast<const wu32x4*>(dst + dimg + nb * G::D_BYTES + p * 4096);
+            Oct8<true> o;
+            o.q = make_uint4(q.x, q.y, q.z, q.w);
+            float v[8];
+            oct8_f8(o, v);
+#pragma unroll
+            for (int j = 0; j < 8; ++j) dbs[nb][j] += v[j];
+          }
+      }
+    }
     if constexpr (R1 < GP) {
       constexpr int R2 = R1 + RB < GP ? R1 + RB : GP;
       static_for<R1, R2>([&](auto pc) { load_g(pc, gbase, iz0, iy0); });
@@ -269,26 +344,38 @@
       }
     }
     __syncthreads();
+    if constexpr (DMA) {
+      dtgt = DIMG - dimg;
+      issue(min(tile + 1, t1 - 1));
+    } else {
     if (tile + 1 < t1) issue(tile + 1);
+    }
+#define MMTTA_TR_FRAG_T(ptr, off) (DMA ? wtr_frag_scoped((ptr), (off)) : MMTTA_TR_FRAG((ptr), (off)))
     constexpr int LA = 3, NF = G::NK * 7;
     wbf16x8 ra[LA + 1], fb[2][NB];
 #pragma unroll
-    for (int nb = 0; nb < NB; ++nb) fb[0][nb] = MMTTA_TR_FRAG(dread, nb * G::D_BYTES);
-#pragma unroll
-    for (int f = 0; f < LA; ++f) ra[f] = MMTTA_TR_FRAG(gread[f % 7], G::row_off(f / 7));
+    for (int nb = 0; nb < NB; ++nb) fb[0][nb] = MMTTA_TR_FRAG_T(DMA ? dcur : dread, nb * G::D_BYTES);
+#pragma unroll
+    for (int f = 0; f < LA; ++f) ra[f] = MMTTA_TR_FRAG_T(gread[f % 7], G::row_off(f / 7));
     __builtin_amdgcn_sched_barrier(0);
 #pragma unroll
     for (int f = 0; f < NF; ++f) {
       const int ks = f / 7, j = f % 7;
-      if (f + LA < NF) ra[(f + LA) % (LA + 1)] = MMTTA_TR_FRAG(gread[(f + LA) % 7], G::row_off((f + LA) / 7));
+      if (f + LA < NF) ra[(f + LA) % (LA + 1)] = MMTTA_TR_FRAG_T(gread[(f + LA) % 7], G::row_off((f + LA) / 7));
       if (j == 2 && ks + 1 < G::NK) {
 #pragma unroll
-        for (int nb = 0; nb < NB; ++nb) fb[(ks + 1) & 1][nb] = MMTTA_TR_FRAG(dread, nb * G::D_BYTES + (ks + 1) * 1024);
+        for (int nb = 0; nb < NB; ++nb) fb[(ks + 1) & 1][nb] = MMTTA_TR_FRAG_T(DMA ? dcur : dread, nb * G::D_BYTES + (ks + 1) * 1024);
       }
 #pragma unroll
       for (int nb = 0; nb < NB; ++nb)
         acc[nb][j] = __builtin_amdgcn_mfma_f32_32x32x16_bf16(ra[f % (LA + 1)], fb[ks & 1][nb], acc[nb][j], 0, 0, 0);
       __builtin_amdgcn_sched_barrier(0);
+    }
+#undef MMTTA_TR_FRAG_T
+    if constexpr (DMA) {
+      asm volatile("s_waitcnt vmcnt(0)" ::: "memory");
+      dcur += DIMG - 2 * dimg;
+      dimg = DIMG - dimg;
     }
     __syncthreads();
   }
```
